# ugadiarov-la-phystech-edu/OCRL

Hardware: AMD Instinct MI355X
Metric: images/sec (node) SLATE pretrain 128x128, 6 slots, 3 iters (higher is better)
Workload: dtype f32

## Files before the change

include/ocrl_hip.h:

```cpp
#ifndef OCRL_HIP_H
#define OCRL_HIP_H
#include <stddef.h>

#ifdef __cplusplus
extern "C" {
#endif

#define OCRL_ABI_VERSION 5

const char* ocrl_last_error(void);
int ocrl_abi_version(void);

typedef struct ocrl_slate ocrl_slate;
typedef struct ocrl_slate_config {
    int obs_size, obs_channels;
    int vocab_size, d_model;
    int cnn_hidden;
    int num_slots, num_iterations, slot_size, mlp_hidden;
    int num_dec_blocks, num_dec_heads;
    float dropout;
    int max_batch;
    int use_bcdec;
    int hard;
    int num_slot_heads;
// ... 1 lines not shown

size_t ocrl_slate_config_size(void);
int ocrl_slate_create(const ocrl_slate_config* cfg, ocrl_slate** out);
void ocrl_slate_destroy(ocrl_slate* h);

int ocrl_slate_param_count(const ocrl_slate* h);
int ocrl_slate_param_info(const ocrl_slate* h, int i, char* name, int name_cap, int shape[4], int* ndim,
                          long long* offset, long long* numel, int* group);
long long ocrl_slate_flat_size(const ocrl_slate* h);
long long ocrl_slate_group_begin(const ocrl_slate* h, int group);
size_t ocrl_slate_workspace_bytes(const ocrl_slate* h);

int ocrl_slate_bind(ocrl_slate* h, float* params, float* grads, float* adam_m, float* adam_v, void* workspace, size_t workspace_bytes);

int ocrl_slate_forward(ocrl_slate* h, const float* obs, int B, float tau, int train, unsigned long long seed,
                       const float* noise_z, const float* noise_zh, const float* noise_slots, void* stream);
int ocrl_slate_backward(ocrl_slate* h, void* stream);
int ocrl_slate_encode(ocrl_slate* h, const float* obs, int B, unsigned long long seed, const float* noise_slots, void* stream);
int ocrl_slate_encode_backward(ocrl_slate* h, const float* dslots, void* stream);
int ocrl_slate_freeze_weights(ocrl_slate* h, int on);
int ocrl_slate_generate(ocrl_slate* h, void* stream);
int ocrl_slate_clip_adam(ocrl_slate* h, const float lr[3], float clip, int step, float grad_scale, void* stream);
int ocrl_slate_grad_norm(ocrl_slate* h, void* stream);
float* ocrl_slate_metrics(const ocrl_slate* h);
int ocrl_slate_tensor(const ocrl_slate* h, const char* name, float** ptr, long long* count);
int ocrl_slate_soft_z(ocrl_slate* h, void* stream);
int ocrl_slate_dropout_mask(const ocrl_slate* h, unsigned site, long long n, float* out, void* stream);

int ocrl_gemm(const float* A, const float* B, float* C, int M, int N, int K, int lda, int ldb, int ldc, int akc, int bkc,
              float alpha, const float* bias, int relu, const float* mask, int ldmask, const float* resid, int ldr,
              int splitk, float* ws, void* stream);
typedef struct ocrl_gemm_desc {
    const float* A; const float* B; float* C;
    int M, N, K, lda, ldb, ldc;
    int akc, bkc;
    int batch, batch_inner;
    long long sA, sB, sC, sAi, sBi, sCi;
    int splitk; float alpha;
    const float* bias; int relu;
    float drop_p; unsigned long long drop_seed; unsigned drop_site;
    const float* mask; int ldmask; long long sMask; int mask_elu;
    const float* resid; int ldr; long long sR;
    float adrop_p; unsigned adrop_site; int adrop_ld;
    float* bias_out; long long sBias;
    int a_mode, b_mode; const float* x_lse; const int* x_tok; float x_scale;
    int epi_mode; float* stat; float* hstat; int* hidx; const float* e1; const float* e2; unsigned long long e_seed;
    const float* e_lse; const float* e_rowvec; float e_scale;
    int force_tile, force_sb;
} ocrl_gemm_desc;
size_t ocrl_gemm_desc_size(void);
int ocrl_gemm_ex(const ocrl_gemm_desc* d, float* ws, size_t ws_floats, void* stream);
int ocrl_gemm_plan(const ocrl_gemm_desc* d, int out[6]);
int ocrl_conv2d_fwd(const float* x, const float* w, const float* bias, float* y, int B, int H, int W, int cin, int cin_pad, int ks,
                    int relu, float* ws, void* stream);
int ocrl_conv2d_fwd_lowlat(const float* x, const float* w, const float* bias, float* y, int B, int H, int W, int cin, int cin_pad, int ks,
                           int relu, float* ws, void* stream);
size_t ocrl_conv2d_x3_ws_floats(void);
int ocrl_conv2d_fwd_x3(const float* x, const float* w, const float* bias, float* y, int B, int H, int W, int ks, int relu, float* ws, void* stream);
int ocrl_conv2d_bwd_data_x3(const float* dy, const float* w, const float* mask, float* dx, int B, int H, int W, int ks, float* ws, void* stream);
int ocrl_conv2d_bwd_weight_x3(const float* x, const float* dy, float* dw, int B, int H, int W, int ks, float* ws, size_t ws_floats, void* stream);
int ocrl_conv2d_bwd_data(const float* dy, const float* w, const float* mask, float* dx, int B, int H, int W, int ks, float* ws, void* stream);
size_t ocrl_conv2d_wgrad_ws_floats(int B, int H, int W, int ks, int cin_pad);
int ocrl_conv2d_bwd_weight(const float* x, const float* dy, float* dw, float* db, int B, int H, int W, int cin, int cin_pad, int ks,
                           float* ws, size_t ws_floats, void* stream);
typedef struct ocrl_conv_desc {
    const float* x; const float* w; float* y;
    int B, H, W, cin, cin_pad, ks;
    const float* bias; int relu;
    const float* posmap; const float* mask; int mask_elu;
    int transposed, low_latency;
} ocrl_conv_desc;
size_t ocrl_conv_desc_size(void);
int ocrl_conv2d_ex(const ocrl_conv_desc* d, float* ws, size_t ws_floats, void* stream);
typedef struct ocrl_conv_wgrad_desc {
    const float* x; const float* dy; float* dw; float* db;
    int B, H, W, cin, cin_pad, ks;
    int accumulate;
} ocrl_conv_wgrad_desc;
size_t ocrl_conv_wgrad_desc_size(void);
int ocrl_conv2d_bwd_weight_ex(const ocrl_conv_wgrad_desc* d, float* ws, size_t ws_floats, void* stream);
int ocrl_layernorm_fwd(const float* x, const float* gamma, const float* beta, float* y, float* mean, float* rstd, long long R, int F, void* stream);
int ocrl_layernorm_bwd(const float* dy, const float* x, const float* mean, const float* rstd, const float* gamma, float* dx, float* dgb,
                       long long R, int F, float* ws, size_t ws_floats, void* stream);

int ocrl_sa_input_plan(long long R, int out[3]);
int ocrl_sa_input_fwd(const float* e4, const float* gamma, const float* beta, const float* W0, const float* b0, const float* W2, const float* b2,
                      float* mean, float* rstd, float* h1, float* x, long long R, int max_wgs, void* stream);
int ocrl_sa_input_bwd(const float* dx, const float* h1, const float* e4, const float* mean, const float* rstd, const float* gamma, const float* beta,
                      const float* W0, const float* W2, float* de4, float* dW0, float* db0, float* dW2, float* db2, float* dgamma, float* dbeta,
                      long long R, int max_wgs, float* ws, size_t ws_floats, void* stream);

int ocrl_attention_fwd(const float* q, const float* k, const float* v, float* o, float* lse, int B, int T, int d, int h, int ld,
                       float p, unsigned long long seed, unsigned site, void* stream);
int ocrl_attention_bwd(const float* q, const float* k, const float* v, const float* o, const float* lse, const float* dO,
                       float* dq, float* dk, float* dv, float* delta, int B, int T, int d, int h, int ld,
                       float p, unsigned long long seed, unsigned site, void* stream);

int ocrl_obs_u8_to_f32(const unsigned char* obs_hwc, float* obs_chw, int B, int H, int W, int C, void* stream);

int ocrl_prof_enable(unsigned tag_mask);
int ocrl_prof_collect(double* ms, long long* count, int ntags);

size_t ocrl_slot_attention_ws_floats(int B, int K, int D, int H, int I);
int ocrl_slot_attention_fwd(const float* x, const float* slots0, const float* const* w, float* slots, float* attn, int B, int N, int K, int D,
                            int H, int I, float* ws, size_t ws_floats, void* stream);
int ocrl_slot_attention_bwd(const float* x, const float* dslots, float* dx, float* dslots0, float* const* dw, int B, int N, int K, int D, int H,
                            int I, float* ws, size_t ws_floats, void* stream);
size_t ocrl_slot_attention_mh_ws_floats(int B, int N, int K, int D, int H, int I, int heads);
int ocrl_slot_attention_mh_fwd(const float* x, const float* slots0, const float* const* w, float* slots, float* attn, int B, int N, int K, int D,
                               int H, int I, int heads, float* ws, size_t ws_floats, void* stream);
int ocrl_slot_attention_mh_bwd(const float* x, const float* dslots, float* dx, float* dslots0, float* const* dw, int B, int N, int K, int D, int H,
                               int I, int heads, float* ws, size_t ws_floats, void* stream);
int ocrl_slot_attention_plan(int K, int D, int H, int heads, int* out6);

#define OCRL_POOL_MAX_LAYERS 8
size_t ocrl_pool_transformer_ws_floats(int B, int K, int d, int nhead, int ff, int L);
int ocrl_pool_transformer_fwd(const float* slots, const float* const* w, const float* pos, float* out, int B, int K, int Din, int d, int nhead,
                              int ff, int L, float drop_p, unsigned long long seed, float* ws, size_t ws_floats, void* stream);
int ocrl_pool_transformer_bwd(const float* slots, const float* dout, const float* const* w, float* dslots, float* const* dw, int B, int K, int Din,
                              int d, int nhead, int ff, int L, float drop_p, unsigned long long seed, float* ws, size_t ws_floats, void* stream);
int ocrl_pool_transformer_dropout_mask(int layer, int which, long long n, float drop_p, unsigned long long seed, float* out, void* stream);
size_t ocrl_pool_transformer_long_ws_floats(int B, int K, int Din, int d, int nhead, int ff, int L);
int ocrl_pool_transformer_long_fwd(const float* slots, const float* const* w, const float* pos, float* out, int B, int K, int Din, int d, int nhead,
                                   int ff, int L, float drop_p, unsigned long long seed, float* ws, size_t ws_floats, void* stream);
int ocrl_pool_transformer_long_bwd(const float* slots, const float* dout, const float* const* w, float* dslots, float* const* dw, int B, int K,
                                   int Din, int d, int nhead, int ff, int L, float drop_p, unsigned long long seed, float* ws, size_t ws_floats,
                                   void* stream);

#define OCRL_POOL_RN_MAX_LAYERS 16
size_t ocrl_pool_rn_ws_floats(int B, int K, int D, int ng, const int* g_dims, int nf, const int* f_dims);
int ocrl_pool_rn_fwd(const float* slots, const float* const* w, float* out, int B, int K, int D, int ng, const int* g_dims, int nf, const int* f_dims,
                     float* ws, size_t ws_floats, void* stream);
int ocrl_pool_rn_bwd(const float* slots, const float* dout, const float* const* w, float* dslots, float* const* dw, int B, int K, int D, int ng,
                     const int* g_dims, int nf, const int* f_dims, float* ws, size_t ws_floats, void* stream);

#define OCRL_NATURECNN_MAX_GROUPS 16
#define OCRL_NATURECNN_MAX_CONVS 4
size_t ocrl_naturecnn_ws_floats(int B, int H, int W, int cin, int groups, int cnn_feat_size, int use_cnn_feat, int rep_dim);
int ocrl_naturecnn_fwd(const float* obs, const float* const* w, float* out, int B, int H, int W, int cin, int groups, int cnn_feat_size,
                       int use_cnn_feat, int rep_dim, int save, float* ws, size_t ws_floats, void* stream);
int ocrl_naturecnn_bwd(const float* obs, const float* dout, const float* const* w, float* const* dw, int B, int H, int W, int cin, int groups,
                       int cnn_feat_size, int use_cnn_feat, int rep_dim, float* ws, size_t ws_floats, void* stream);

size_t ocrl_pool_cnn_ws_floats(int B, int H, int W, int D, int rep_dim);
int ocrl_pool_cnn_fwd(const float* tokens, const float* const* w, float* out, int B, int H, int W, int D, int rep_dim, int save, float* ws,
                      size_t ws_floats, void* stream);
int ocrl_pool_cnn_bwd(const float* tokens, const float* dout, const float* const* w, float* dtokens, float* const* dw, int B, int H, int W, int D,
                      int rep_dim, float* ws, size_t ws_floats, void* stream);

#define OCRL_VAE_MAX_STAGES 6
size_t ocrl_vae_ws_floats(int B, int obs_size, int obs_channels, int cnn_feat_size, int latent_dim, int use_cnn_feat, int full);
int ocrl_vae_fwd(const float* obs, const float* const* w, const float* eps, float* rep, float* metrics, float* recon, int B, int obs_size,
                 int obs_channels, int cnn_feat_size, int latent_dim, int use_cnn_feat, float kld_weight, int full, float* ws, size_t ws_floats,
                 void* stream);
int ocrl_vae_bwd(const float* obs, const float* eps, const float* const* w, const float* dloss, const float* drep, float* const* dw, int B,
                 int obs_size, int obs_channels, int cnn_feat_size, int latent_dim, int use_cnn_feat, float kld_weight, int full, float* ws,
                 size_t ws_floats, void* stream);

#define OCRL_MAE_MAX_DEPTH 32
size_t ocrl_mae_ws_floats(int B, int obs_size, int patch, int D, int depth, int heads, int Dd, int ddepth, int dheads, int len_keep, int full);
int ocrl_mae_fwd(const float* obs, const float* const* w, const float* noise, float* rep, float* metrics, float* pred, float* mask,
                 int* ids_restore, int B, int obs_size, int patch, int D, int depth, int heads, int Dd, int ddepth, int dheads, int len_keep,
                 int full, float* ws, size_t ws_floats, void* stream);
int ocrl_mae_bwd(const float* obs, const float* const* w, const float* dloss, const float* drep, float* const* dw, int B, int obs_size,
                 int patch, int D, int depth, int heads, int Dd, int ddepth, int dheads, int len_keep, int full, float* ws, size_t ws_floats,
                 void* stream);
// ... 119 lines not shown
```

ocrl_amd/_lib.py:

```python
import ctypes
import os
from ctypes import POINTER, c_char_p, c_float, c_int, c_longlong, c_size_t, c_uint, c_ulonglong, c_void_p

_HERE = os.path.dirname(os.path.abspath(__file__))
LIB_PATH = os.environ.get("OCRL_HIP_LIB") or os.path.join(_HERE, "libocrl_hip.so")
_lib = None


class SlateConfig(ctypes.Structure):
    _fields_ = [(n, c_int) for n in ("obs_size", "obs_channels", "vocab_size", "d_model", "cnn_hidden", "num_slots",
                                      "num_iterations", "slot_size", "mlp_hidden", "num_dec_blocks", "num_dec_heads")] + \
               [("dropout", c_float), ("max_batch", c_int), ("use_bcdec", c_int), ("hard", c_int), ("num_slot_heads", c_int)]


class IodineConfig(ctypes.Structure):
    _fields_ = [(n, c_int) for n in ("obs_size", "obs_channels", "slot_size", "num_iterations", "num_slots")] + \
               [("sigma", c_float), ("beta", c_float), ("layer_norm", c_int), ("ref_mlp_hidden", c_int), ("max_batch", c_int)]


class GemmDesc(ctypes.Structure):
    _fields_ = [("A", c_void_p), ("B", c_void_p), ("C", c_void_p)] + \
               [(n, c_int) for n in ("M", "N", "K", "lda", "ldb", "ldc", "akc", "bkc", "batch", "batch_inner")] + \
               [(n, c_longlong) for n in ("sA", "sB", "sC", "sAi", "sBi", "sCi")] + \
               [("splitk", c_int), ("alpha", c_float), ("bias", c_void_p), ("relu", c_int),
# ... 51 lines not shown


def conv_desc(**kw):
    d = ConvDesc()
    for k, v in kw.items():
        setattr(d, k, v)
    return d


def conv_wgrad_desc(**kw):
    d = ConvWgradDesc()
    for k, v in kw.items():
        setattr(d, k, v)
    return d


def lib():
    global _lib
    if _lib is not None:
        return _lib
    if not os.path.exists(LIB_PATH):
        raise RuntimeError(
            f"{LIB_PATH} is missing: build it with `python -c 'import __graft_entry__ as g; g.build()'` "
            "(make -C ocrl_amd/csrc).  ocrl_amd has no CPU fallback.")
    import torch
    L = ctypes.CDLL(LIB_PATH)
    p = c_void_p
    L.ocrl_last_error.restype = c_char_p
    L.ocrl_abi_version.restype = c_int
    L.ocrl_slate_config_size.restype = c_size_t
    if L.ocrl_slate_config_size() != ctypes.sizeof(SlateConfig):
        raise RuntimeError(f"libocrl_hip.so: ocrl_slate_config is {L.ocrl_slate_config_size()} bytes, this binding's SlateConfig {ctypes.sizeof(SlateConfig)}")
    L.ocrl_slate_create.argtypes = [POINTER(SlateConfig), POINTER(p)]
    L.ocrl_slate_destroy.argtypes = [p]
    L.ocrl_slate_destroy.restype = None
    L.ocrl_slate_param_count.argtypes = [p]
    L.ocrl_slate_param_info.argtypes = [p, c_int, c_char_p, c_int, POINTER(c_int * 4), POINTER(c_int), POINTER(c_longlong),
                                        POINTER(c_longlong), POINTER(c_int)]
    L.ocrl_slate_flat_size.argtypes = [p]
    L.ocrl_slate_flat_size.restype = c_longlong
    L.ocrl_slate_group_begin.argtypes = [p, c_int]
    L.ocrl_slate_group_begin.restype = c_longlong
    L.ocrl_slate_workspace_bytes.argtypes = [p]
    L.ocrl_slate_workspace_bytes.restype = c_size_t
    L.ocrl_slate_bind.argtypes = [p, p, p, p, p, p, c_size_t]
    L.ocrl_slate_forward.argtypes = [p, p, c_int, c_float, c_int, c_ulonglong, p, p, p, p]
    L.ocrl_slate_backward.argtypes = [p, p]
    L.ocrl_slate_generate.argtypes = [p, p]
    L.ocrl_slate_encode.argtypes = [p, p, c_int, c_ulonglong, p, p]
    L.ocrl_slate_encode_backward.argtypes = [p, p, p]
    L.ocrl_slate_freeze_weights.argtypes = [p, c_int]
    L.ocrl_slate_clip_adam.argtypes = [p, POINTER(c_float * 3), c_float, c_int, c_float, p]
    L.ocrl_slate_grad_norm.argtypes = [p, p]
    L.ocrl_slate_metrics.argtypes = [p]
    L.ocrl_slate_metrics.restype = p
    L.ocrl_slate_tensor.argtypes = [p, c_char_p, POINTER(p), POINTER(c_longlong)]
    L.ocrl_slate_dropout_mask.argtypes = [p, c_uint, c_longlong, p, p]
    L.ocrl_slate_soft_z.argtypes = [p, p]
    L.ocrl_gemm.argtypes = [p, p, p, c_int, c_int, c_int, c_int, c_int, c_int, c_int, c_int, c_float, p, c_int, p, c_int, p, c_int,
                            c_int, p, p]
    L.ocrl_gemm_desc_size.restype = c_size_t
    L.ocrl_gemm_ex.argtypes = [POINTER(GemmDesc), p, c_size_t, p]
    L.ocrl_gemm_plan.argtypes = [POINTER(GemmDesc), POINTER(c_int * 6)]
    L.ocrl_conv2d_fwd.argtypes = [p, p, p, p, c_int, c_int, c_int, c_int, c_int, c_int, c_int, p, p]
    L.ocrl_conv2d_fwd_lowlat.argtypes = [p, p, p, p, c_int, c_int, c_int, c_int, c_int, c_int, c_int, p, p]
    L.ocrl_conv2d_x3_ws_floats.restype = c_size_t
    L.ocrl_conv2d_fwd_x3.argtypes = [p, p, p, p, c_int, c_int, c_int, c_int, c_int, p, p]
    L.ocrl_conv2d_bwd_data_x3.argtypes = [p, p, p, p, c_int, c_int, c_int, c_int, p, p]
    L.ocrl_conv2d_bwd_weight_x3.argtypes = [p, p, p, c_int, c_int, c_int, c_int, p, c_size_t, p]
    L.ocrl_conv2d_bwd_data.argtypes = [p, p, p, p, c_int, c_int, c_int, c_int, p, p]
    L.ocrl_conv2d_wgrad_ws_floats.argtypes = [c_int, c_int, c_int, c_int, c_int]
    L.ocrl_conv2d_wgrad_ws_floats.restype = c_size_t
    L.ocrl_conv2d_bwd_weight.argtypes = [p, p, p, p, c_int, c_int, c_int, c_int, c_int, c_int, p, c_size_t, p]
    L.ocrl_conv_desc_size.restype = c_size_t
    L.ocrl_conv_wgrad_desc_size.restype = c_size_t
    for name, cls in (("ocrl_conv_desc", ConvDesc), ("ocrl_conv_wgrad_desc", ConvWgradDesc)):
        n = getattr(L, name + "_size")()
        if n != ctypes.sizeof(cls):
            raise RuntimeError(f"libocrl_hip.so: {name} is {n} bytes, this binding's {cls.__name__} {ctypes.sizeof(cls)}")
    L.ocrl_conv2d_ex.argtypes = [POINTER(ConvDesc), p, c_size_t, p]
    L.ocrl_conv2d_bwd_weight_ex.argtypes = [POINTER(ConvWgradDesc), p, c_size_t, p]
    L.ocrl_layernorm_fwd.argtypes = [p, p, p, p, p, p, c_longlong, c_int, p]
    L.ocrl_layernorm_bwd.argtypes = [p, p, p, p, p, p, p, c_longlong, c_int, p, c_size_t, p]
    L.ocrl_sa_input_plan.argtypes = [c_longlong, POINTER(c_int * 3)]
    L.ocrl_sa_input_fwd.argtypes = [p] * 11 + [c_longlong, c_int, p]
    L.ocrl_sa_input_bwd.argtypes = [p] * 16 + [c_longlong, c_int, p, c_size_t, p]
    L.ocrl_attention_fwd.argtypes = [p, p, p, p, p, c_int, c_int, c_int, c_int, c_int, c_float, c_ulonglong, c_uint, p]
    L.ocrl_attention_bwd.argtypes = [p, p, p, p, p, p, p, p, p, p, c_int, c_int, c_int, c_int, c_int, c_float, c_ulonglong, c_uint, p]
    L.ocrl_obs_u8_to_f32.argtypes = [p, p, c_int, c_int, c_int, c_int, p]
    L.ocrl_prof_enable.argtypes = [c_uint]
    L.ocrl_prof_collect.argtypes = [POINTER(ctypes.c_double * 8), POINTER(c_longlong * 8), c_int]
    L.ocrl_iodine_create.argtypes = [POINTER(IodineConfig), POINTER(p)]
    L.ocrl_iodine_destroy.argtypes = [p]
    L.ocrl_iodine_destroy.restype = None
    L.ocrl_iodine_param_count.argtypes = [p]
    L.ocrl_iodine_param_info.argtypes = [p, c_int, c_char_p, c_int, POINTER(c_int * 4), POINTER(c_int), POINTER(c_longlong), POINTER(c_longlong)]
    L.ocrl_iodine_flat_size.argtypes = [p]
    L.ocrl_iodine_flat_size.restype = c_longlong
    L.ocrl_iodine_workspace_bytes.argtypes = [p]
    L.ocrl_iodine_workspace_bytes.restype = c_size_t
    L.ocrl_iodine_bind.argtypes = [p, p, p, p, p, p, c_size_t]
    L.ocrl_iodine_forward.argtypes = [p, p, c_int, c_ulonglong, p, p]
    L.ocrl_iodine_backward.argtypes = [p, p]
    L.ocrl_iodine_clip_adam.argtypes = [p, c_float, c_float, c_int, c_float, p]
    L.ocrl_iodine_grad_norm.argtypes = [p, p]
    L.ocrl_iodine_metrics.argtypes = [p]
    L.ocrl_iodine_metrics.restype = p
    L.ocrl_iodine_tensor.argtypes = [p, c_char_p, POINTER(p), POINTER(c_longlong)]
    L.ocrl_slot_attention_ws_floats.argtypes = [c_int, c_int, c_int, c_int, c_int]
    L.ocrl_slot_attention_ws_floats.restype = c_size_t
    L.ocrl_slot_attention_fwd.argtypes = [p, p, POINTER(p), p, p, c_int, c_int, c_int, c_int, c_int, c_int, p, c_size_t, p]
    L.ocrl_slot_attention_bwd.argtypes = [p, p, p, p, POINTER(p), c_int, c_int, c_int, c_int, c_int, c_int, p, c_size_t, p]
    L.ocrl_slot_attention_mh_ws_floats.argtypes = [c_int] * 7
    L.ocrl_slot_attention_mh_ws_floats.restype = c_size_t
    L.ocrl_slot_attention_mh_fwd.argtypes = [p, p, POINTER(p), p, p] + [c_int] * 7 + [p, c_size_t, p]
    L.ocrl_slot_attention_mh_bwd.argtypes = [p, p, p, p, POINTER(p)] + [c_int] * 7 + [p, c_size_t, p]
    L.ocrl_slot_attention_plan.argtypes = [c_int, c_int, c_int, c_int, POINTER(c_int * 6)]
    L.ocrl_pool_transformer_ws_floats.argtypes = [c_int, c_int, c_int, c_int, c_int, c_int]
    L.ocrl_pool_transformer_ws_floats.restype = c_size_t
    L.ocrl_pool_transformer_fwd.argtypes = [p, POINTER(p), p, p, c_int, c_int, c_int, c_int, c_int, c_int, c_int, c_float, c_ulonglong, p, c_size_t, p]
    L.ocrl_pool_transformer_bwd.argtypes = [p, p, POINTER(p), p, POINTER(p), c_int, c_int, c_int, c_int, c_int, c_int, c_int, c_float, c_ulonglong, p,
                                            c_size_t, p]
    L.ocrl_pool_transformer_dropout_mask.argtypes = [c_int, c_int, c_longlong, c_float, c_ulonglong, p, p]
    L.ocrl_pool_transformer_long_ws_floats.argtypes = [c_int] * 7
    L.ocrl_pool_transformer_long_ws_floats.restype = c_size_t
    L.ocrl_pool_transformer_long_fwd.argtypes = L.ocrl_pool_transformer_fwd.argtypes
    L.ocrl_pool_transformer_long_bwd.argtypes = L.ocrl_pool_transformer_bwd.argtypes
    L.ocrl_pool_rn_ws_floats.argtypes = [c_int, c_int, c_int, c_int, POINTER(c_int), c_int, POINTER(c_int)]
    L.ocrl_pool_rn_ws_floats.restype = c_size_t
    L.ocrl_pool_rn_fwd.argtypes = [p, POINTER(p), p, c_int, c_int, c_int, c_int, POINTER(c_int), c_int, POINTER(c_int), p, c_size_t, p]
    L.ocrl_pool_rn_bwd.argtypes = [p, p, POINTER(p), p, POINTER(p), c_int, c_int, c_int, c_int, POINTER(c_int), c_int, POINTER(c_int), p, c_size_t, p]
    L.ocrl_naturecnn_ws_floats.argtypes = [c_int] * 8
    L.ocrl_naturecnn_ws_floats.restype = c_size_t
    L.ocrl_naturecnn_fwd.argtypes = [p, POINTER(p), p] + [c_int] * 9 + [p, c_size_t, p]
    L.ocrl_naturecnn_bwd.argtypes = [p, p, POINTER(p), POINTER(p)] + [c_int] * 8 + [p, c_size_t, p]
    L.ocrl_pool_cnn_ws_floats.argtypes = [c_int] * 5
    L.ocrl_pool_cnn_ws_floats.restype = c_size_t
    L.ocrl_pool_cnn_fwd.argtypes = [p, POINTER(p), p] + [c_int] * 6 + [p, c_size_t, p]
    L.ocrl_pool_cnn_bwd.argtypes = [p, p, POINTER(p), p, POINTER(p)] + [c_int] * 5 + [p, c_size_t, p]
    L.ocrl_vae_ws_floats.argtypes = [c_int] * 7
    L.ocrl_vae_ws_floats.restype = c_size_t
    L.ocrl_vae_fwd.argtypes = [p, POINTER(p), p, p, p, p] + [c_int] * 6 + [c_float, c_int, p, c_size_t, p]
    L.ocrl_vae_bwd.argtypes = [p, p, POINTER(p), p, p, POINTER(p)] + [c_int] * 6 + [c_float, c_int, p, c_size_t, p]
    L.ocrl_mae_ws_floats.argtypes = [c_int] * 11
    L.ocrl_mae_ws_floats.restype = c_size_t
    L.ocrl_mae_fwd.argtypes = [p, POINTER(p), p, p, p, p, p, p] + [c_int] * 11 + [p, c_size_t, p]
    L.ocrl_mae_bwd.argtypes = [p, POINTER(p), p, p, POINTER(p)] + [c_int] * 11 + [p, c_size_t, p]
    L.ocrl_mae_rank.argtypes = [p, p, p, p, c_int, c_int, c_int, p]
    L.ocrl_probe_ws_floats.argtypes = [c_int] * 7 + [POINTER(c_int), c_int]
    L.ocrl_probe_ws_floats.restype = c_size_t
    L.ocrl_probe_fwd.argtypes = [p, POINTER(p), p, p, p, p, p] + [c_int] * 8 + [POINTER(c_int), c_float, c_int, POINTER(c_int), POINTER(c_int),
                                 POINTER(c_int), p, c_size_t, p]
    L.ocrl_probe_bwd.argtypes = [p, p, POINTER(p), POINTER(p)] + [c_int] * 7 + [POINTER(c_int), c_float, c_int, p, c_size_t, p]
    L.ocrl_probe_match_ws_floats.argtypes = [c_int, c_int]
    L.ocrl_probe_match_ws_floats.restype = c_size_t
    L.ocrl_probe_match.argtypes = [p, c_int, c_longlong, p, p, p, p, p, p] + [c_int] * 6 + [POINTER(c_int)] * 3 + [p, c_size_t, p]
    L.ocrl_ari_counts.argtypes = [p, c_longlong, c_longlong, c_longlong, c_int, p, c_longlong, c_longlong, c_longlong, c_int, c_int, c_int, c_longlong, p, p, p]
    L.ocrl_acnet_desc_size.restype = c_size_t
    if L.ocrl_acnet_desc_size() != ctypes.sizeof(AcnetDesc):
        raise RuntimeError(f"libocrl_hip.so: ocrl_acnet_desc is {L.ocrl_acnet_desc_size()} bytes, this binding's AcnetDesc {ctypes.sizeof(AcnetDesc)}")
    L.ocrl_acnet_ws_floats.argtypes = [POINTER(AcnetDesc)]
    L.ocrl_acnet_ws_floats.restype = c_size_t
    L.ocrl_acnet_fwd.argtypes = [POINTER(AcnetDesc), p, POINTER(p), p, p, p, p, c_int, p, c_size_t, p]
    L.ocrl_acnet_bwd.argtypes = [POINTER(AcnetDesc), p, POINTER(p), p, p, p, p, p, POINTER(p), p, c_size_t, p]
    L.ocrl_acnet_ppo_fwd_bwd.argtypes = [POINTER(AcnetDesc), p, POINTER(p), p, p, p, p, c_float, c_float, c_float, c_int, p, p, POINTER(p), p, c_size_t, p]
    L.ocrl_acnet_a2c_fwd_bwd.argtypes = [POINTER(AcnetDesc), p, POINTER(p), p, p, p, c_float, c_float, c_int, p, p, POINTER(p), p, c_size_t, p]
# ... 48 lines not shown
```

ocrl_amd/csrc/capi.cpp:

```cpp
#include <stdarg.h>
#include <stdint.h>
#include <string.h>

#include <new>

#include "../../include/ocrl_hip.h"
#include "iodine_model.h"
#include "slate_model.h"

static thread_local char g_err[512] = "";

void ocrl_set_error(const char* fmt, ...) {
    va_list ap;
    va_start(ap, fmt);
    vsnprintf(g_err, sizeof g_err, fmt, ap);
    va_end(ap);
}

template <class M>
struct Handle {
    using Model = M;
    M* m = nullptr;
};
struct ocrl_slate : Handle<SlateModel> {};
// ... 193 lines not shown
    if (conv_pack_x3_launch(w, ws, nullptr, ST(stream), ks)) return 1;
    ConvArgs a;
    a.X = x; a.Y = y; a.B = B; a.H = H; a.W = W; a.bias = bias; a.relu = relu;
    return conv_x3_launch(a, ws, ST(stream), ks);
}
int ocrl_conv2d_bwd_data_x3(const float* dy, const float* w, const float* mask, float* dx, int B, int H, int W, int ks, float* ws, void* stream) {
    if (ks != 3 && ks != 5) { ocrl_set_error("ocrl_conv2d_bwd_data_x3: ks must be 3 or 5"); return 1; }
    if (conv_pack_x3_launch(w, ws, ws + conv_x3_pack_floats(5), ST(stream), ks)) return 1;
    ConvArgs a;
    a.X = dy; a.Y = dx; a.B = B; a.H = H; a.W = W; a.mask = mask;
    return conv_x3_launch(a, ws + conv_x3_pack_floats(5), ST(stream), ks);
}
int ocrl_conv2d_bwd_data(const float* dy, const float* w, const float* mask, float* dx, int B, int H, int W, int ks, float* ws, void* stream) {
    float* bw = ws + (size_t)ks * ks * 64 * 64;
    if (conv_pack_launch(w, ws, bw, ks, 64, 64, 64, ST(stream))) return 1;
    ConvArgs a;
    a.X = dy; a.Wp = bw; a.Y = dx; a.B = B; a.H = H; a.W = W; a.mask = mask;
    return conv_fwd_launch(a, ks, 64, 64, ST(stream));
}
size_t ocrl_conv2d_wgrad_ws_floats(int B, int H, int W, int ks, int cin_pad) { return conv_wgrad_ws_floats(B, H, W, ks, cin_pad) + (1 << 16); }
int ocrl_conv2d_bwd_weight(const float* x, const float* dy, float* dw, float* db, int B, int H, int W, int cin, int cin_pad, int ks, float* ws,
                           size_t ws_floats, void* stream) {
    if (ws_floats < ocrl_conv2d_wgrad_ws_floats(B, H, W, ks, cin_pad)) { ocrl_set_error("ocrl_conv2d_bwd_weight: workspace too small"); return 1; }
    WgradArgs a;
    a.X = x; a.dY = dy; a.part = ws; a.B = B; a.H = H; a.W = W;
    if (conv_wgrad_launch(a, ks, cin_pad, 64, cin, dw, 0, ST(stream), 0)) return 1;
    if (db) return colsum_launch(dy, 64, db, (long long)B * H * W, 64, 0, 1.f, ws, ws_floats, ST(stream));
    return 0;
}
int ocrl_conv2d_bwd_weight_x3(const float* x, const float* dy, float* dw, int B, int H, int W, int ks, float* ws, size_t ws_floats, void* stream) {
    if (ks != 3 && ks != 5) { ocrl_set_error("ocrl_conv2d_bwd_weight_x3: ks must be 3 or 5"); return 1; }
    if (ws_floats < ocrl_conv2d_wgrad_ws_floats(B, H, W, ks, 64)) { ocrl_set_error("ocrl_conv2d_bwd_weight_x3: workspace too small"); return 1; }
    WgradArgs a;
    a.X = x; a.dY = dy; a.part = ws; a.B = B; a.H = H; a.W = W;
    return conv_wgrad_launch(a, ks, 64, 64, 64, dw, 0, ST(stream), 1);
}
static bool conv_kernel_built(int ks, int cin_pad) { return (ks == 5 && (cin_pad == 64 || cin_pad == 8)) || (ks == 3 && cin_pad == 64); }
static bool aligned16(const void* p) { return ((uintptr_t)p & 15) == 0; }
size_t ocrl_conv_desc_size(void) { return sizeof(ocrl_conv_desc); }
int ocrl_conv2d_ex(const ocrl_conv_desc* d, float* ws, size_t ws_floats, void* stream) {
    if (!d) { ocrl_set_error("ocrl_conv2d_ex: null descriptor"); return 1; }
    if (!d->x || !d->w || !d->y || !ws || d->B < 1 || d->H < 1 || d->W < 1) { ocrl_set_error("ocrl_conv2d_ex: x, w, y, ws and a non-empty image are required"); return 1; }
    if (!conv_kernel_built(d->ks, d->cin_pad)) { ocrl_set_error("ocrl_conv2d_ex: no kernel for ks=%d cin_pad=%d (built: 5/64, 5/8, 3/64)", d->ks, d->cin_pad); return 1; }
    if (d->cin < 1 || d->cin > d->cin_pad) { ocrl_set_error("ocrl_conv2d_ex: cin %d outside 1 .. cin_pad %d", d->cin, d->cin_pad); return 1; }
    if (d->relu < 0 || d->relu > 2) { ocrl_set_error("ocrl_conv2d_ex: relu must be 0, 1 (ReLU) or 2 (ELU), got %d", d->relu); return 1; }
    if (d->mask_elu && !d->mask) { ocrl_set_error("ocrl_conv2d_ex: mask_elu needs a mask"); return 1; }
    if (d->transposed && (d->cin != 64 || d->cin_pad != 64)) { ocrl_set_error("ocrl_conv2d_ex: the transposed (backward-data) form needs cin = cin_pad = 64"); return 1; }
    if (!aligned16(d->x) || !aligned16(d->y) || !aligned16(ws) || !aligned16(d->bias) || !aligned16(d->posmap) || !aligned16(d->mask)) {
        ocrl_set_error("ocrl_conv2d_ex: x, y, ws, bias, posmap and mask must be 16-byte aligned");
        return 1;
    }
    const size_t pack = (size_t)d->ks * d->ks * d->cin_pad * 64, need = d->transposed ? 2 * pack : pack;
    if (ws_floats < need) { ocrl_set_error("ocrl_conv2d_ex: workspace of %zu floats, %zu needed", ws_floats, need); return 1; }
    float* bw = d->transposed ? ws + pack : nullptr;
    if (conv_pack_launch(d->w, ws, bw, d->ks, d->cin_pad, 64, d->cin, ST(stream))) return 1;
    ConvArgs a;
    a.X = d->x; a.Wp = bw ? bw : ws; a.Y = d->y; a.B = d->B; a.H = d->H; a.W = d->W; a.bias = d->bias; a.relu = d->relu;
    a.posmap = d->posmap; a.mask = d->mask; a.mask_elu = d->mask_elu ? 1 : 0;
    return conv_fwd_launch(a, d->ks, d->cin_pad, 64, ST(stream), d->low_latency ? 1 : 0);
}
size_t ocrl_conv_wgrad_desc_size(void) { return sizeof(ocrl_conv_wgrad_desc); }
int ocrl_conv2d_bwd_weight_ex(const ocrl_conv_wgrad_desc* d, float* ws, size_t ws_floats, void* stream) {
    if (!d) { ocrl_set_error("ocrl_conv2d_bwd_weight_ex: null descriptor"); return 1; }
    if (!d->x || !d->dy || !d->dw || !ws || d->B < 1 || d->H < 1 || d->W < 1) { ocrl_set_error("ocrl_conv2d_bwd_weight_ex: x, dy, dw, ws and a non-empty image are required"); return 1; }
    if (!conv_kernel_built(d->ks, d->cin_pad)) { ocrl_set_error("ocrl_conv2d_bwd_weight_ex: no kernel for ks=%d cin_pad=%d (built: 5/64, 5/8, 3/64)", d->ks, d->cin_pad); return 1; }
    if (d->cin < 1 || d->cin > d->cin_pad) { ocrl_set_error("ocrl_conv2d_bwd_weight_ex: cin %d outside 1 .. cin_pad %d", d->cin, d->cin_pad); return 1; }
    if (!aligned16(d->x) || !aligned16(d->dy) || !aligned16(ws)) { ocrl_set_error("ocrl_conv2d_bwd_weight_ex: x, dy and ws must be 16-byte aligned"); return 1; }
    const size_t need = ocrl_conv2d_wgrad_ws_floats(d->B, d->H, d->W, d->ks, d->cin_pad);
    if (ws_floats < need) { ocrl_set_error("ocrl_conv2d_bwd_weight_ex: workspace of %zu floats, %zu needed", ws_floats, need); return 1; }
    const int acc = d->accumulate ? 1 : 0;
    WgradArgs a;
    a.X = d->x; a.dY = d->dy; a.part = ws; a.B = d->B; a.H = d->H; a.W = d->W;
    if (conv_wgrad_launch(a, d->ks, d->cin_pad, 64, d->cin, d->dw, acc, ST(stream), 0)) return 1;
    if (d->db) return colsum_launch(d->dy, 64, d->db, (long long)d->B * d->H * d->W, 64, acc, 1.f, ws, ws_floats, ST(stream));
    return 0;
}
int ocrl_layernorm_fwd(const float* x, const float* g, const float* b, float* y, float* mean, float* rstd, long long R, int F, void* stream) {
    return layernorm_fwd_launch(x, g, b, y, mean, rstd, R, F, ST(stream));
}
int ocrl_layernorm_bwd(const float* dy, const float* x, const float* mean, const float* rstd, const float* g, float* dx, float* dgb, long long R,
                       int F, float* ws, size_t ws_floats, void* stream) {
    return layernorm_bwd_launch(dy, x, mean, rstd, g, dx, dgb, R, F, 0, 0, ws, ws_floats, ST(stream));
}

int ocrl_sa_input_plan(long long R, int out[3]) {
    if (!out || R <= 0) { ocrl_set_error("ocrl_sa_input_plan: needs R > 0 and an output array"); return 1; }
    sa_input_plan(R, 0, out);
    return 0;
}
int ocrl_sa_input_fwd(const float* e4, const float* gamma, const float* beta, const float* W0, const float* b0, const float* W2, const float* b2,
                      float* mean, float* rstd, float* h1, float* x, long long R, int max_wgs, void* stream) {
    return sa_input_fwd_launch(e4, gamma, beta, W0, b0, W2, b2, mean, rstd, nullptr, h1, x, R, max_wgs, ST(stream));
}
int ocrl_sa_input_bwd(const float* dx, const float* h1, const float* e4, const float* mean, const float* rstd, const float* gamma, const float* beta,
                      const float* W0, const float* W2, float* de4, float* dW0, float* db0, float* dW2, float* db2, float* dgamma, float* dbeta,
                      long long R, int max_wgs, float* ws, size_t ws_floats, void* stream) {
    return sa_input_bwd_launch(dx, h1, e4, mean, rstd, gamma, beta, W0, W2, de4, dW0, db0, dW2, db2, dgamma, dbeta, R, max_wgs, ws, ws_floats,
                               ST(stream));
}

int ocrl_attention_fwd(const float* q, const float* k, const float* v, float* o, float* lse, int B, int T, int d, int h, int ld, float p,
                       unsigned long long seed, unsigned site, void* stream) {
    AttnArgs a;
    a.q = q; a.k = k; a.v = v; a.o = o; a.lse = lse; a.B = B; a.T = T; a.d = d; a.h = h; a.ld = ld; a.p = p; a.seed = seed; a.site = site;
    return attn_launch(a, 0, ST(stream));
}
int ocrl_attention_bwd(const float* q, const float* k, const float* v, const float* o, const float* lse, const float* dO, float* dq,
                       float* dk, float* dv, float* delta, int B, int T, int d, int h, int ld, float p, unsigned long long seed,
                       unsigned site, void* stream) {
    AttnArgs a;
    a.q = q; a.k = k; a.v = v; a.o = const_cast<float*>(o); a.lse = const_cast<float*>(lse); a.B = B; a.T = T; a.d = d; a.h = h; a.ld = ld;
    a.p = p; a.seed = seed; a.site = site; a.dO = dO; a.dq = dq; a.dk = dk; a.dv = dv; a.delta = delta;
    return attn_launch(a, 1, ST(stream));
}


int ocrl_iodine_create(const ocrl_iodine_config* c, ocrl_iodine** out) {
    if (!c || !out) { ocrl_set_error("ocrl_iodine_create: null argument"); return 1; }
    if (c->obs_size < 16 || c->obs_size % 16 || c->obs_channels != 3 || c->slot_size < 4 || c->slot_size % 4 || c->slot_size > 256 ||
        c->num_iterations < 1 || c->num_slots < 1 || c->num_slots > 16 || c->ref_mlp_hidden < 64 || c->ref_mlp_hidden % 64 || c->max_batch < 1 ||
        !(c->sigma > 0.f)) {
        ocrl_set_error("ocrl_iodine_create: invalid configuration");
        return 1;
    }
    IodineConfig k;
    k.obs_size = c->obs_size; k.obs_channels = c->obs_channels; k.slot_size = c->slot_size; k.num_iters = c->num_iterations;
    k.num_slots = c->num_slots; k.sigma = c->sigma; k.beta = c->beta; k.layer_norm = c->layer_norm; k.ref_mlp_hidden = c->ref_mlp_hidden;
    k.max_batch = c->max_batch;
    return h_create(k, out);
}
void ocrl_iodine_destroy(ocrl_iodine* h) { h_destroy(h); }
int ocrl_iodine_param_count(const ocrl_iodine* h) { return h_param_count(h); }
int ocrl_iodine_param_info(const ocrl_iodine* h, int i, char* name, int name_cap, int shape[4], int* ndim, long long* offset, long long* numel) {
    return h_param_info(h, i, name, name_cap, shape, ndim, offset, numel, nullptr);
}
long long ocrl_iodine_flat_size(const ocrl_iodine* h) { return h_flat_size(h); }
size_t ocrl_iodine_workspace_bytes(const ocrl_iodine* h) { return h_workspace_bytes(h); }
int ocrl_iodine_bind(ocrl_iodine* h, float* p, float* g, float* m, float* v, void* ws, size_t n) { return h_bind(h, p, g, m, v, ws, n); }
int ocrl_iodine_forward(ocrl_iodine* h, const float* obs, int B, unsigned long long seed, const float* noise, void* stream) {
    GUARD(h);
    return h->m->forward(obs, B, seed, noise, ST(stream));
}
int ocrl_iodine_backward(ocrl_iodine* h, void* stream) { GUARD(h); return h->m->backward(ST(stream)); }
int ocrl_iodine_clip_adam(ocrl_iodine* h, float lr, float clip, int step, float gscale, void* stream) {
    GUARD(h);
    return h->m->clip_adam(lr, clip, step, gscale, ST(stream));
}
int ocrl_iodine_grad_norm(ocrl_iodine* h, void* stream) { GUARD(h); return h->m->grad_norm(ST(stream)); }
float* ocrl_iodine_metrics(const ocrl_iodine* h) { return h_metrics(h); }
int ocrl_iodine_tensor(const ocrl_iodine* h, const char* name, float** ptr, long long* count) { return h_tensor(h, name, ptr, count); }
}
```

ocrl_amd/csrc/elementwise.hip:

```cpp
#include "common.h"
#include "kernels.h"
#include "layernorm16.h"

#define TINYF 1.17549435e-38f

__device__ inline float block_sum(float v, float* red) {
    v = wave_sum(v);
    const int w = threadIdx.x >> 6, nw = blockDim.x >> 6;
    __syncthreads();
    if ((threadIdx.x & 63) == 0) red[w] = v;
    __syncthreads();
    float s = 0.f;
    for (int i = 0; i < nw; ++i) s += red[i];
    return s;
}
__device__ inline float block_max(float v, float* red) {
    v = wave_max(v);
    const int w = threadIdx.x >> 6, nw = blockDim.x >> 6;
    __syncthreads();
    if ((threadIdx.x & 63) == 0) red[w] = v;
    __syncthreads();
    float s = red[0];
    for (int i = 1; i < nw; ++i) s = fmaxf(s, red[i]);
    return s;
// ... 74 lines not shown
        const int c = i * 64 + lane;
        y[row * F + c] = (v[i] - mu) * rs * g[c] + bta[c];
    }
    if (lane == 0) {
        if (mean) mean[row] = mu;
        if (rstd) rstd[row] = rs;
    }
}

template <int NPL>
__global__ void layernorm_bwd_kernel(const float* __restrict__ dy, const float* __restrict__ x, const float* __restrict__ mean,
                                     const float* __restrict__ rstd, const float* __restrict__ g, float* __restrict__ dx,
                                     float* __restrict__ part, long long R, int accumulate) {
    constexpr int F = 64 * NPL;
    __shared__ float red[4][2 * F];
    const int lane = threadIdx.x & 63, wv = threadIdx.x >> 6;
    float dg[NPL], db[NPL], gg[NPL];
#pragma unroll
    for (int i = 0; i < NPL; ++i) { dg[i] = 0.f; db[i] = 0.f; gg[i] = g[i * 64 + lane]; }
    for (long long row = (long long)blockIdx.x * 4 + wv; row < R; row += (long long)gridDim.x * 4) {
        const float mu = mean[row], rs = rstd[row];
        float xh[NPL], d[NPL];
        float s1 = 0.f, s2 = 0.f;
#pragma unroll
        for (int i = 0; i < NPL; ++i) {
            const int c = i * 64 + lane;
            xh[i] = (x[row * F + c] - mu) * rs;
            const float dyv = dy[row * F + c];
            dg[i] += dyv * xh[i];
            db[i] += dyv;
            d[i] = dyv * gg[i];
            s1 += d[i];
            s2 += d[i] * xh[i];
        }
        s1 = wave_sum(s1) * (1.0f / F);
        s2 = wave_sum(s2) * (1.0f / F);
#pragma unroll
        for (int i = 0; i < NPL; ++i) {
            const int c = i * 64 + lane;
            const float v = rs * (d[i] - s1 - xh[i] * s2);
            dx[row * F + c] = accumulate ? dx[row * F + c] + v : v;
        }
    }
#pragma unroll
    for (int i = 0; i < NPL; ++i) { red[wv][i * 64 + lane] = dg[i]; red[wv][F + i * 64 + lane] = db[i]; }
    __syncthreads();
    for (int c = threadIdx.x; c < 2 * F; c += blockDim.x)
        part[(size_t)blockIdx.x * 2 * F + c] = red[0][c] + red[1][c] + red[2][c] + red[3][c];
}

template <int NV, int NP>
__global__ __launch_bounds__(256) void layernorm16_fwd_kernel(const float* __restrict__ x, const float* __restrict__ g, const float* __restrict__ bta,
                                                              float* __restrict__ y, float* __restrict__ mean, float* __restrict__ rstd, long long R) {
    constexpr int F = 64 * NV;
    const int lane = threadIdx.x & 63, wv = threadIdx.x >> 6, c4 = lane & 15, rsub = lane >> 4;
    const long long row0 = ((long long)blockIdx.x * 4 + wv) * (4 * NP) + rsub;
    float4 v[NP][NV];
#pragma unroll
    for (int i = 0; i < NP; ++i)
#pragma unroll
        for (int k = 0; k < NV; ++k) {
            const long long row = row0 + 4 * i;
            v[i][k] = row < R ? *reinterpret_cast<const float4*>(x + row * F + (k * 16 + c4) * 4) : make_float4(0.f, 0.f, 0.f, 0.f);
        }
    float4 gg[NV], bb[NV];
#pragma unroll
    for (int k = 0; k < NV; ++k) { gg[k] = *reinterpret_cast<const float4*>(g + (k * 16 + c4) * 4); bb[k] = *reinterpret_cast<const float4*>(bta + (k * 16 + c4) * 4); }
#pragma unroll
    for (int i = 0; i < NP; ++i) {
        const long long row = row0 + 4 * i;
        float mu, rs;
        layernorm16_row_fwd<NV>(v[i], mu, rs);
        if (row < R) {
#pragma unroll
            for (int k = 0; k < NV; ++k) *reinterpret_cast<float4*>(y + row * F + (k * 16 + c4) * 4) = layernorm16_affine(v[i][k], rs, gg[k], bb[k]);
            if (c4 == 0) {
                if (mean) mean[row] = mu;
                if (rstd) rstd[row] = rs;
            }
        }
    }
}
template <int NV, int NP>
__global__ __launch_bounds__(256) void layernorm16_bwd_kernel(const float* __restrict__ dy, const float* __restrict__ x, const float* __restrict__ mean,
                                                              const float* __restrict__ rstd, const float* __restrict__ g, float* __restrict__ dx,
                                                              float* __restrict__ part, long long R, int accumulate) {
    constexpr int F = 64 * NV;
    __shared__ float4 red[2][16][16 * NV];
    const int lane = threadIdx.x & 63, wv = threadIdx.x >> 6, c4 = lane & 15, rsub = lane >> 4;
    float4 gg[NV], dg[NV], db[NV];
#pragma unroll
    for (int k = 0; k < NV; ++k) { gg[k] = *reinterpret_cast<const float4*>(g + (k * 16 + c4) * 4); dg[k] = make_float4(0.f, 0.f, 0.f, 0.f); db[k] = dg[k]; }
    for (long long grp = blockIdx.x; grp * (16 * NP) < R; grp += gridDim.x) {
        const long long row0 = (grp * 4 + wv) * (4 * NP) + rsub;
        float4 xv[NP][NV], yv[NP][NV];
        float mu[NP], rs[NP];
#pragma unroll
        for (int i = 0; i < NP; ++i) {
            const long long row = row0 + 4 * i;
            const bool ok = row < R;
#pragma unroll
            for (int k = 0; k < NV; ++k) {
                xv[i][k] = ok ? *reinterpret_cast<const float4*>(x + row * F + (k * 16 + c4) * 4) : make_float4(0.f, 0.f, 0.f, 0.f);
                yv[i][k] = ok ? *reinterpret_cast<const float4*>(dy + row * F + (k * 16 + c4) * 4) : make_float4(0.f, 0.f, 0.f, 0.f);
            }
            mu[i] = ok ? mean[row] : 0.f;
            rs[i] = ok ? rstd[row] : 0.f;
        }
#pragma unroll
        for (int i = 0; i < NP; ++i) {
            const long long row = row0 + 4 * i;
            const Ln16Bwd<NV> r = layernorm16_row_bwd<NV>(xv[i], yv[i], mu[i], rs[i], gg, dg, db);
            if (row < R) {
#pragma unroll
                for (int k = 0; k < NV; ++k) {
                    float4 o = layernorm16_row_dx(r, rs[i], k);
                    float* dp = dx + row * F + (k * 16 + c4) * 4;
                    if (accumulate) { const float4 a = *reinterpret_cast<const float4*>(dp); o.x += a.x; o.y += a.y; o.z += a.z; o.w += a.w; }
                    *reinterpret_cast<float4*>(dp) = o;
                }
            }
        }
    }
#pragma unroll
    for (int k = 0; k < NV; ++k) { red[0][wv * 4 + rsub][k * 16 + c4] = dg[k]; red[1][wv * 4 + rsub][k * 16 + c4] = db[k]; }
    __syncthreads();
    if (threadIdx.x < 32 * NV) {
        const int which = threadIdx.x / (16 * NV), c = threadIdx.x % (16 * NV);
        float4 a = red[which][0][c];
#pragma unroll
        for (int k = 1; k < 16; ++k) { const float4 t = red[which][k][c]; a.x += t.x; a.y += t.y; a.z += t.z; a.w += t.w; }
        *reinterpret_cast<float4*>(part + (size_t)blockIdx.x * (2 * F) + which * F + c * 4) = a;
    }
}

__global__ void colsum_kernel(const float* __restrict__ X, long long ld, float* __restrict__ part, long long R, int F, long long rows_per_chunk) {
    __shared__ float red[4][64];
    const int col = blockIdx.x * 64 + (threadIdx.x & 63), rl = threadIdx.x >> 6;
    const long long r0 = (long long)blockIdx.y * rows_per_chunk;
    const long long r1 = min(R, r0 + rows_per_chunk);
    float s = 0.f;
    if (col < F)
        for (long long r = r0 + rl; r < r1; r += 4) s += X[r * ld + col];
    red[rl][threadIdx.x & 63] = s;
    __syncthreads();
    if (rl == 0 && col < F) part[(size_t)blockIdx.y * F + col] = red[0][threadIdx.x] + red[1][threadIdx.x] + red[2][threadIdx.x] + red[3][threadIdx.x];
}
__global__ __launch_bounds__(256) void colsum4_kernel(const float* __restrict__ X, long long ld, float* __restrict__ part, long long R, int F,
                                                      long long rows_per_chunk) {
    __shared__ float4 red[256];
    const int F4 = F >> 2, RL = 256 / F4;
    const int c4 = threadIdx.x % F4, rl = threadIdx.x / F4;
    const long long r0 = (long long)blockIdx.x * rows_per_chunk;
    const long long r1 = min(R, r0 + rows_per_chunk);
    float4 s0 = make_float4(0.f, 0.f, 0.f, 0.f), s1 = s0, s2 = s0, s3 = s0;
    if (rl < RL) {
        const float* base = X + (size_t)c4 * 4;
        long long r = r0 + rl;
        for (; r + 3 * RL < r1; r += 4 * RL) {
            const float4 a = *reinterpret_cast<const float4*>(base + r * ld), b = *reinterpret_cast<const float4*>(base + (r + RL) * ld);
            const float4 c = *reinterpret_cast<const float4*>(base + (r + 2 * RL) * ld), d = *reinterpret_cast<const float4*>(base + (r + 3 * RL) * ld);
            s0.x += a.x; s0.y += a.y; s0.z += a.z; s0.w += a.w;
            s1.x += b.x; s1.y += b.y; s1.z += b.z; s1.w += b.w;
            s2.x += c.x; s2.y += c.y; s2.z += c.z; s2.w += c.w;
            s3.x += d.x; s3.y += d.y; s3.z += d.z; s3.w += d.w;
        }
        for (; r < r1; r += RL) {
            const float4 a = *reinterpret_cast<const float4*>(base + r * ld);
            s0.x += a.x; s0.y += a.y; s0.z += a.z; s0.w += a.w;
        }
    }
    red[threadIdx.x] = make_float4(s0.x + s1.x + s2.x + s3.x, s0.y + s1.y + s2.y + s3.y, s0.z + s1.z + s2.z + s3.z, s0.w + s1.w + s2.w + s3.w);
    __syncthreads();
    if (threadIdx.x < F4) {
        float4 t = red[threadIdx.x];
        for (int k = 1; k < RL; ++k) { const float4 v = red[k * F4 + threadIdx.x]; t.x += v.x; t.y += v.y; t.z += v.z; t.w += v.w; }
        *reinterpret_cast<float4*>(part + (size_t)blockIdx.x * F + threadIdx.x * 4) = t;
    }
}
__global__ __launch_bounds__(256) void colsum_final_kernel(const float* __restrict__ part, float* __restrict__ out, int nchunk, int F, int accumulate, float scale) {
    __shared__ float red[16][16];
    const int cl = threadIdx.x & 15, rl = threadIdx.x >> 4;
    const int c = blockIdx.x * 16 + cl;
    float s0 = 0.f, s1 = 0.f;
    if (c < F) {
        int k = rl;
        for (; k + 16 < nchunk; k += 32) { s0 += part[(size_t)k * F + c]; s1 += part[(size_t)(k + 16) * F + c]; }
        if (k < nchunk) s0 += part[(size_t)k * F + c];
    }
    red[rl][cl] = s0 + s1;
    __syncthreads();
    if (rl == 0 && c < F) {
        float t = 0.f;
#pragma unroll
        for (int k = 0; k < 16; ++k) t += red[k][cl];
        t *= scale;
        out[c] = accumulate ? out[c] + t : t;
    }
}

__global__ void reduce_partials_kernel(const float* __restrict__ part, int n, float* __restrict__ out, float scale, int accumulate) {
    __shared__ float red[4];
    float s = 0.f;
    for (int i = threadIdx.x; i < n; i += blockDim.x) s += part[i];
    s = block_sum(s, red);
    if (threadIdx.x == 0) out[0] = (accumulate ? out[0] : 0.f) + s * scale;
}

__global__ void mse_kernel(const float* __restrict__ obs, const float* __restrict__ recon, float* __restrict__ drecon,
                           float* __restrict__ part, int B, int C, int H, int W, float inv_b) {
    __shared__ float red[4];
    const long long n = (long long)B * H * W, hw = (long long)H * W;
    float s = 0.f;
    for (long long i = (long long)blockIdx.x * blockDim.x + threadIdx.x; i < n; i += (long long)gridDim.x * blockDim.x) {
        const long long b = i / hw, r = i % hw;
        const float4 rc = *reinterpret_cast<const float4*>(recon + i * 4);
        const float rv[4] = {rc.x, rc.y, rc.z, rc.w};
        float d[4] = {0.f, 0.f, 0.f, 0.f};
        for (int c = 0; c < C; ++c) {
            const float e = rv[c] - obs[(b * C + c) * hw + r];
            s += e * e;
            d[c] = 2.f * e * inv_b;
        }
        if (drecon) *reinterpret_cast<float4*>(drecon + i * 4) = make_float4(d[0], d[1], d[2], d[3]);
    }
    s = block_sum(s, red);
    if (threadIdx.x == 0) part[blockIdx.x] = s;
}

#define GS_MAXPT 16
template <int NPT>
__global__ __launch_bounds__(256) void gumbel_softmax_kernel(const float* __restrict__ raw, const float* __restrict__ e1,
                                                             const float* __restrict__ e2, float* __restrict__ z,
                                                             int* __restrict__ tokens, int V, float inv_tau,
                                                             unsigned long long seed, float* __restrict__ zst) {
    __shared__ float red[4];
    __shared__ float redv[4];
    __shared__ int redi[4];
    const long long row = blockIdx.x;
    const float* r = raw + row * V;
    const int npt = NPT ? NPT : V / 256;
    float x[GS_MAXPT];
    float mx = -INFINITY;
#pragma unroll
    for (int i = 0; i < GS_MAXPT; ++i)
        if (i < npt) { x[i] = r[i * 256 + threadIdx.x]; mx = fmaxf(mx, x[i]); }
    mx = block_max(mx, red);
    float s = 0.f;
#pragma unroll
    for (int i = 0; i < GS_MAXPT; ++i)
        if (i < npt) s += __expf(x[i] - mx);
    s = block_sum(s, red);
    const float lse = mx + __logf(s);
    float u[GS_MAXPT];
    float best = -INFINITY;
    int besti = 0;
    float m2 = -INFINITY;
#pragma unroll
    for (int i = 0; i < GS_MAXPT; ++i)
        if (i < npt) {
            const int v = i * 256 + threadIdx.x;
            const float lp = x[i] - lse;
            float ea, eb;
            if (e1) { ea = e1[row * V + v]; eb = e2[row * V + v]; }
            else {
                const uint64_t idx = (uint64_t)row * V + v;
                const uint2 ba = rng_bits4(seed, SITE_GUMBEL_Z, idx);
                ea = -__logf(u01_24(ba.x));
                eb = -__logf(u01_24(ba.y));
            }
            const float g1 = -__logf(ea + TINYF), g2 = -__logf(eb + TINYF);
            u[i] = (lp + g1) * inv_tau;
            m2 = fmaxf(m2, u[i]);
            const float h = (lp + g2) * inv_tau;
            if (h > best) { best = h; besti = v; }
        }
    m2 = block_max(m2, red);
    float s2 = 0.f;
#pragma unroll
    for (int i = 0; i < GS_MAXPT; ++i)
        if (i < npt) { u[i] = __expf(u[i] - m2); s2 += u[i]; }
// ... 741 lines not shown
    if (tid < dh) qs[tid] = base[(size_t)t * ld + tid] * scale;
    __syncthreads();
    float mx = -INFINITY;
    for (int j = tid; j < nk; j += 256) {
        const float* kr = base + (size_t)j * ld + d;
        float a = 0.f;
        for (int c = 0; c < dh; c += 4) {
            const float4 kv = *reinterpret_cast<const float4*>(kr + c);
            a += qs[c] * kv.x + qs[c + 1] * kv.y + qs[c + 2] * kv.z + qs[c + 3] * kv.w;
        }
        sc[j] = a;
        mx = fmaxf(mx, a);
    }
    red[tid] = mx;
    __syncthreads();
    block_tree_max<256>(red);
    mx = red[0];
    __syncthreads();
    float sum = 0.f;
    for (int j = tid; j < nk; j += 256) { const float e = __expf(sc[j] - mx); sc[j] = e; sum += e; }
    red[tid] = sum;
    __syncthreads();
    block_tree_sum<256>(red);
    const float inv = 1.0f / red[0];
    __syncthreads();
    const int nsl = 256 / dh, c = tid % dh, sl = tid / dh;
    float acc = 0.f;
    if (sl < nsl)
        for (int j = sl; j < nk; j += nsl) acc += sc[j] * base[(size_t)j * ld + 2 * d + c];
    red[tid] = sl < nsl ? acc : 0.f;
    __syncthreads();
    if (tid < dh) {
        float a = 0.f;
        for (int k = 0; k < nsl; ++k) a += red[k * dh + tid];
        out[(size_t)b * d + hd * dh + tid] = a * inv;
    }
}

__global__ void onehot_kernel(const int* __restrict__ tokens, float* __restrict__ z, long long n, int V) {
    const long long i = (long long)blockIdx.x * blockDim.x + threadIdx.x;
    if (i >= n) return;
    z[i] = (int)(i % V) == tokens[i / V] ? 1.f : 0.f;
}

int nchw_to_nhwc8_launch(const float* in, float* out, int B, int C, int H, int W, hipStream_t st) {
    OCRL_REQUIRE(C <= 8, "nchw_to_nhwc8: C must be <= 8");
    const long long n = (long long)B * H * W;
    hipLaunchKernelGGL(nchw_to_nhwc8_kernel, GRID1D(n), 0, st, in, out, B, C, H, W);
    OCRL_CHECK_LAUNCH("nchw_to_nhwc8");
    return 0;
}
int patchify4_launch(const float* in, float* out, int B, int C, int S, hipStream_t st) {
    OCRL_REQUIRE(S % 4 == 0, "patchify4: S %% 4 != 0");
    const long long n = (long long)B * (S / 4) * (S / 4) * C * 4;
    hipLaunchKernelGGL(patchify4_kernel, GRID1D(n), 0, st, in, out, B, C, S);
    OCRL_CHECK_LAUNCH("patchify4");
    return 0;
}
int pixel_shuffle_launch(const float* in, float* out, int B, int h, int w, int Cout, int forward, const float* mask, hipStream_t st) {
    const long long n = (long long)B * h * w * Cout;
    hipLaunchKernelGGL(pixel_shuffle_kernel, GRID1D(n), 0, st, in, out, B, h, w, Cout, forward, mask);
    OCRL_CHECK_LAUNCH("pixel_shuffle");
    return 0;
}
int layernorm_fwd_launch(const float* x, const float* g, const float* b, float* y, float* mean, float* rstd, long long R, int F, hipStream_t st) {
    OCRL_REQUIRE(F % 64 == 0 && F >= 64 && F <= 256, "layernorm: F must be 64..256, multiple of 64 (got %d)", F);
    dim3 grid(cdiv(R, 4)), blk(256);
    const bool al16 = aligned16(x, y, g, b);
    switch (F / 64) {
        case 1:
            if (al16) hipLaunchKernelGGL((layernorm16_fwd_kernel<1, 4>), dim3((unsigned)cdiv(R, 64)), blk, 0, st, x, g, b, y, mean, rstd, R);
            else hipLaunchKernelGGL(layernorm_fwd_kernel<1>, grid, blk, 0, st, x, g, b, y, mean, rstd, R);
            break;
        case 2: hipLaunchKernelGGL(layernorm_fwd_kernel<2>, grid, blk, 0, st, x, g, b, y, mean, rstd, R); break;
        case 3:
            if (al16) hipLaunchKernelGGL((layernorm16_fwd_kernel<3, 2>), dim3((unsigned)cdiv(R, 32)), blk, 0, st, x, g, b, y, mean, rstd, R);
            else hipLaunchKernelGGL(layernorm_fwd_kernel<3>, grid, blk, 0, st, x, g, b, y, mean, rstd, R);
            break;
        default: hipLaunchKernelGGL(layernorm_fwd_kernel<4>, grid, blk, 0, st, x, g, b, y, mean, rstd, R); break;
    }
    OCRL_CHECK_LAUNCH("layernorm_fwd");
    return 0;
}
int colsum_launch(const float* X, long long ld, float* out, long long R, int F, int accumulate, float scale, float* ws, size_t ws_floats, hipStream_t st) {
    if (F % 4 == 0 && ld % 4 == 0 && F <= 1024 && F >= 4 && (((uintptr_t)X) & 15) == 0 && R >= 1024) {
        long long nchunk = 2048;
        if (nchunk > R / 8) nchunk = R / 8;
        if ((size_t)nchunk * F > ws_floats) nchunk = (long long)(ws_floats / F);
        if (nchunk >= 16) {
            const long long rpc = (R + nchunk - 1) / nchunk;
            nchunk = (R + rpc - 1) / rpc;
            hipLaunchKernelGGL(colsum4_kernel, dim3((unsigned)nchunk), dim3(256), 0, st, X, ld, ws, R, F, rpc);
            OCRL_CHECK_LAUNCH("colsum4");
            hipLaunchKernelGGL(colsum_final_kernel, dim3(cdiv(F, 16)), dim3(256), 0, st, ws, out, (int)nchunk, F, accumulate, scale);
            OCRL_CHECK_LAUNCH("colsum_final");
            return 0;
        }
    }
    const int cb = cdiv(F, 64);
    long long nchunk = 1024 / cb;
    if (nchunk < 1) nchunk = 1;
    if (nchunk > (R + 63) / 64) nchunk = (R + 63) / 64;
    if (nchunk < 1) nchunk = 1;
    OCRL_REQUIRE((size_t)nchunk * F <= ws_floats, "colsum: workspace too small (%lld x %d)", nchunk, F);
    const long long rpc = (R + nchunk - 1) / nchunk;
    hipLaunchKernelGGL(colsum_kernel, dim3(cb, (int)nchunk), dim3(256), 0, st, X, ld, ws, R, F, rpc);
    OCRL_CHECK_LAUNCH("colsum");
    hipLaunchKernelGGL(colsum_final_kernel, dim3(cdiv(F, 16)), dim3(256), 0, st, ws, out, (int)nchunk, F, accumulate, scale);
    OCRL_CHECK_LAUNCH("colsum_final");
    return 0;
}
int layernorm_bwd_launch(const float* dy, const float* x, const float* mean, const float* rstd, const float* g, float* dx,
                         float* dgb, long long R, int F, int accumulate_dx, int accumulate_dgb, float* ws, size_t ws_floats, hipStream_t st) {
    OCRL_REQUIRE(F % 64 == 0 && F >= 64 && F <= 256, "layernorm bwd: F must be 64..256, multiple of 64 (got %d)", F);
    int nblk = (int)((R + 3) / 4);
    if (nblk > 2048) nblk = 2048;
    while (nblk > 64 && (size_t)nblk * 2 * F * 2 + (size_t)8 * 2 * F > ws_floats) nblk /= 2;
    const size_t need = (size_t)nblk * 2 * F;
    OCRL_REQUIRE(need + (size_t)8 * 2 * F <= ws_floats, "layernorm bwd: workspace too small");
    dim3 grid(nblk), blk(256);
    const bool al16 = aligned16(x, dy, dx, g, ws);
    switch (F / 64) {
        case 1:
            if (al16) hipLaunchKernelGGL((layernorm16_bwd_kernel<1, 4>), grid, blk, 0, st, dy, x, mean, rstd, g, dx, ws, R, accumulate_dx);
            else hipLaunchKernelGGL(layernorm_bwd_kernel<1>, grid, blk, 0, st, dy, x, mean, rstd, g, dx, ws, R, accumulate_dx);
            break;
        case 2: hipLaunchKernelGGL(layernorm_bwd_kernel<2>, grid, blk, 0, st, dy, x, mean, rstd, g, dx, ws, R, accumulate_dx); break;
        case 3:
            if (al16) hipLaunchKernelGGL((layernorm16_bwd_kernel<3, 2>), grid, blk, 0, st, dy, x, mean, rstd, g, dx, ws, R, accumulate_dx);
            else hipLaunchKernelGGL(layernorm_bwd_kernel<3>, grid, blk, 0, st, dy, x, mean, rstd, g, dx, ws, R, accumulate_dx);
            break;
        default: hipLaunchKernelGGL(layernorm_bwd_kernel<4>, grid, blk, 0, st, dy, x, mean, rstd, g, dx, ws, R, accumulate_dx); break;
    }
    OCRL_CHECK_LAUNCH("layernorm_bwd");
    return colsum_launch(ws, 2 * F, dgb, nblk, 2 * F, accumulate_dgb, 1.f, ws + need, ws_floats - need, st);
}
int reduce_partials_launch(const float* part, int n, float* out, float scale, int accumulate, hipStream_t st) {
    hipLaunchKernelGGL(reduce_partials_kernel, dim3(1), dim3(256), 0, st, part, n, out, scale, accumulate);
    OCRL_CHECK_LAUNCH("reduce_partials");
    return 0;
}
int mse_launch(const float* obs, const float* recon, float* drecon, float* out, int B, int C, int H, int W, float* ws, size_t ws_floats, hipStream_t st) {
    OCRL_REQUIRE(C <= 4, "mse: C must be <= 4");
    const int nblk = 1024;
    OCRL_REQUIRE(ws_floats >= (size_t)nblk, "mse: workspace too small");
    hipLaunchKernelGGL(mse_kernel, dim3(nblk), dim3(256), 0, st, obs, recon, drecon, ws, B, C, H, W, 1.0f / B);
    OCRL_CHECK_LAUNCH("mse");
    return reduce_partials_launch(ws, nblk, out, 1.0f / B, 0, st);
}
int gumbel_softmax_launch(const float* raw, const float* e1, const float* e2, float* z, int* tokens, long long R, int V, float tau,
                          unsigned long long seed, hipStream_t st, float* zst) {
    OCRL_REQUIRE(V % 256 == 0 && V <= 256 * GS_MAXPT, "gumbel_softmax: V must be a multiple of 256, <= %d", 256 * GS_MAXPT);
    OCRL_REQUIRE((e1 == nullptr) == (e2 == nullptr), "gumbel_softmax: give both noise tensors or none");
    switch (V / 256) {
        case 16: hipLaunchKernelGGL(gumbel_softmax_kernel<16>, dim3((unsigned)R), dim3(256), 0, st, raw, e1, e2, z, tokens, V, 1.0f / tau, seed, zst); break;
        case 8: hipLaunchKernelGGL(gumbel_softmax_kernel<8>, dim3((unsigned)R), dim3(256), 0, st, raw, e1, e2, z, tokens, V, 1.0f / tau, seed, zst); break;
        default: hipLaunchKernelGGL(gumbel_softmax_kernel<0>, dim3((unsigned)R), dim3(256), 0, st, raw, e1, e2, z, tokens, V, 1.0f / tau, seed, zst); break;
    }
    OCRL_CHECK_LAUNCH("gumbel_softmax");
    return 0;
}
int softmax_bwd_rows_launch(const float* z, float* d, long long R, int V, float scale, hipStream_t st) {
    OCRL_REQUIRE(V % 256 == 0 && V <= 256 * GS_MAXPT, "softmax_bwd_rows: V must be a multiple of 256, <= %d", 256 * GS_MAXPT);
    if (V == 4096) hipLaunchKernelGGL(softmax_bwd_rows_kernel<16>, dim3((unsigned)R), dim3(256), 0, st, z, d, V, scale);
    else hipLaunchKernelGGL(softmax_bwd_rows_kernel<0>, dim3((unsigned)R), dim3(256), 0, st, z, d, V, scale);
    OCRL_CHECK_LAUNCH("softmax_bwd_rows");
    return 0;
}
int softmax_stat_combine_launch(const float* stat, int nseg, long long R, float* lse, const float* hstat, const int* hidx, int* tokens,
                                const float* pred, int ldp, const int* tok, float* out, float scale, float* ws, size_t ws_floats, hipStream_t st,
                                const float* cdf_scores, int cdf_V, float cdf_tau, unsigned long long cdf_seed) {
    OCRL_REQUIRE(nseg >= 1 && nseg <= 64, "softmax_stat_combine: 1..64 segments (got %d)", nseg);
    const long long nblk = (R + 15) / 16;
    OCRL_REQUIRE(!pred || (tok && out && ws && ws_floats >= (size_t)nblk), "softmax_stat_combine: cross-entropy needs tokens, an output and %lld workspace floats", nblk);
    CdfArgs cdf;
    cdf.scores = cdf_scores; cdf.V = cdf_V; cdf.tau = cdf_tau; cdf.seed = cdf_seed;
    OCRL_REQUIRE(!cdf_scores || (hstat && hidx && tokens && cdf_V > 0 && cdf_V <= nseg * 64), "softmax_stat_combine: inverse-CDF sampling arguments");
    hipLaunchKernelGGL(softmax_stat_combine_kernel, dim3((unsigned)nblk), dim3(1024), 0, st, stat, nseg, R, lse, hstat, hidx, tokens, pred, ldp, tok,
                       pred ? ws : nullptr, cdf);
    OCRL_CHECK_LAUNCH("softmax_stat_combine");
    if (pred) return reduce_partials_launch(ws, (int)nblk, out, scale, 0, st);
    return 0;
}
int exp_rows_launch(const float* y, const float* lse, float* z, long long R, int V, hipStream_t st) {
    OCRL_REQUIRE(V % 4 == 0, "exp_rows: V %% 4 != 0");
    const long long n4 = R * (V / 4);
    hipLaunchKernelGGL(exp_rows_kernel, dim3((unsigned)((n4 + 255) / 256)), dim3(256), 0, st, y, lse, z, n4, V / 4);
    OCRL_CHECK_LAUNCH("exp_rows");
    return 0;
}
int rowdot_bias64_launch(const float* g, const float* act, const float* bias, long long R, float* out, hipStream_t st) {
    OCRL_REQUIRE(((((uintptr_t)g) | ((uintptr_t)act) | ((uintptr_t)bias)) & 15) == 0, "rowdot: operands must be 16-byte aligned");
    hipLaunchKernelGGL(rowdot_bias64_kernel, dim3((unsigned)((R + 15) / 16)), dim3(256), 0, st, g, act, bias, R, out);
    OCRL_CHECK_LAUNCH("rowdot_bias64");
    return 0;
}
int embed_fwd_launch(const int* tokens, const float* dict, const float* bos, const float* pe, float* out, int B, int T, int d, float p,
                     unsigned long long seed, hipStream_t st) {
    OCRL_REQUIRE(d % 4 == 0, "embed: d %% 4 != 0");
    const long long n = (long long)B * T * (d / 4);
    hipLaunchKernelGGL(embed_fwd_kernel, dim3((unsigned)cdiv(n, 1024)), dim3(256), 0, st, tokens, dict, bos, pe, out, B, T, d, p, seed);
    OCRL_CHECK_LAUNCH("embed_fwd");
    return 0;
}
static size_t eb_align(size_t n) { return (n + 63) & ~(size_t)63; }
size_t embed_bwd_ws_floats(long long BT, int V, int d) {
    const size_t nchunk = (size_t)cdiv(BT, EB_CHUNK), nunit = (size_t)cdiv(BT, EB_UNIT);
    return eb_align(nchunk * (V + 1)) + 2 * eb_align((size_t)V + 2) + eb_align((size_t)BT) + eb_align(nunit * 2 * d);
}
int embed_bwd_launch(float* g, const int* tokens, float* ddict, int B, int T, int V, int d, float p, unsigned long long seed, float* ws,
                     size_t ws_floats, hipStream_t st) {
    const long long BT = (long long)B * T;
    OCRL_REQUIRE(d % 4 == 0 && d <= 1024 && V + 1 <= 16384 && BT < (1ll << 31), "embed_bwd: unsupported shape (d %d, vocabulary %d, %lld rows)", d, V, BT);
    OCRL_REQUIRE(ws && ws_floats >= embed_bwd_ws_floats(BT, V, d), "embed_bwd: scratch too small");
    const int nchunk = cdiv(BT, EB_CHUNK), nunit = cdiv(BT, EB_UNIT);
    int* hist = reinterpret_cast<int*>(ws);
    int* total = hist + eb_align((size_t)nchunk * (V + 1));
    int* base = total + eb_align((size_t)V + 2);
// ... 179 lines not shown
```

ocrl_amd/csrc/kernels.h:

```cpp
#pragma once
#include "common.h"
#include "../../include/ocrl_hip.h"

enum { PROF_CONV5 = 0, PROF_CONV_OTHER = 1, PROF_WGRAD = 2, PROF_GEMM = 3, PROF_SA_FWD = 4, PROF_SA_BWD = 5, PROF_ATTN_FWD = 6, PROF_ATTN_BWD = 7, PROF_NTAGS = 8 };
int prof_begin(int tag, hipStream_t st);
void prof_end(int idx, hipStream_t st);

struct GemmArgs {
    const float* A = nullptr;
    const float* B = nullptr;
    float* C = nullptr;
    int M = 0, N = 0, K = 0;
    int lda = 0, ldb = 0, ldc = 0;
    int akc = 1, bkc = 1;
    int batch = 1;
    int batch_inner = 1;
    long long sA = 0, sB = 0, sC = 0;
    long long sAi = 0, sBi = 0, sCi = 0;
    int splitk = 1;
    long long sCsplit = 0;
    float alpha = 1.f;
    const float* bias = nullptr;
    int relu = 0;
    float drop_p = 0.f;
// ... 121 lines not shown
struct PcDxArgs {
    const float* dY = nullptr; const float* Wd = nullptr; float* dX = nullptr;
    int H = 0, W = 0, D = 0, OH = 0, OW = 0, HB = 0, WT = 0, Dp = 0, passes = 0, upw = 0;
    long long units = 0, groups = 0;
};
int pc_conv1_fwd_launch(const float* X, const float* w, const float* bias, float* Wp, float* Y, int B, int H, int W, int D, hipStream_t st);
int pc_conv1_dw_launch(const float* X, const float* dY, float* part, int B, int H, int W, int D, hipStream_t st);
int pc_conv1_dw_reduce_launch(const float* part, float* dw, float* db, int B, int H, int W, int D, hipStream_t st);
int pc_conv1_dx_launch(const float* dY, const float* w, float* Wd, float* dX, int B, int H, int W, int D, hipStream_t st);

#define PROBE_MAX_SLOTS 12
#define PROBE_MAX_PROPS 8
#define PROBE_MAX_WIDTH 256
struct ProbeSchema { int P; int t[PROBE_MAX_PROPS], a[PROBE_MAX_PROPS], b[PROBE_MAX_PROPS], kind[PROBE_MAX_PROPS]; };
int probe_schema_check(const ProbeSchema& sc, int T, int O);
int probe_match_check(int B, int K, int N, int T, int O);
int probe_match_launch(const float* out, int ld_row, long long ld_img, const float* y, const float* dloss, float* cost, int* col, float* part,
                       float* metrics, float* dout, int B, int K, int N, int T, int O, const ProbeSchema& sc, hipStream_t st);
int probe_leaky_fwd_launch(float* x, long long n, float slope, hipStream_t st);
int probe_leaky_bwd_launch(float* dx, const float* h, long long n, float slope, hipStream_t st);

int vae_permute_launch(const float* src, float* dst, long long R, int C, int HW, int rows, int pack, hipStream_t st);
int vae_pad_rows_launch(const float* src, float* dst, int rows, int rows_pad, int K, hipStream_t st);
int vae_kl_fwd_launch(const float* ml, const float* eps, float* latent, float* part, float* rep, int B, int L, hipStream_t st);
int vae_loss_launch(const float* part, float* metrics, int B, float kld_weight, hipStream_t st);
int vae_kl_bwd_launch(const float* ml, const float* eps, const float* dlat, const float* drep, const float* dloss, float* dml, int B, int L,
                      float kld_weight, hipStream_t st);
int vae_scale_launch(const float* x, float* y, const float* g, long long n, hipStream_t st);
int vae_recon_nchw_launch(const float* r4, float* out, int B, int C, int HW, hipStream_t st);

#define MAE_MAX_PATCHES 1024
int mae_rank_launch(const float* noise, int* restore, int* keep, float* mask, int* restore_out, float* mask_out, int B, int L, int len_keep,
                    hipStream_t st);
int mae_patch_gather_launch(const float* obs, const int* ids, float* out, int B, int n, int S, int p, hipStream_t st);
int mae_tokens_fwd_launch(const float* embed, const float* cls, const float* pos, const int* ids, float* x0, int B, int n, int D, hipStream_t st);
int mae_tokens_bwd_launch(const float* dx0, float* dembed, float* dcls, int B, int n, int D, hipStream_t st);
int mae_unshuffle_fwd_launch(const float* e, const float* mtok, const float* dpos, const int* restore, float* xd, int B, int L, int len_keep, int Dd,
                             hipStream_t st);
int mae_unshuffle_bwd_launch(const float* dxd, const int* keep, const float* mask, float* de, float* dmtok, float* part, int B, int L, int len_keep,
                             int Dd, hipStream_t st);
int mae_gelu_fwd_launch(const float* pre, float* y, long long n, hipStream_t st);
int mae_gelu_bwd_launch(const float* dy, const float* pre, float* dpre, long long n, hipStream_t st);
int mae_ln_fwd_launch(const float* x, const float* g, const float* b, float* y, float* mean, float* rstd, long long R, int F, float eps, hipStream_t st);
int mae_ln_chunks(long long R);
int mae_ln_bwd_launch(const float* dy, const float* x, const float* mean, const float* rstd, const float* g, const float* resid, float* dx, float* dg,
                      float* db, float* part, long long R, int F, hipStream_t st);
int mae_loss_launch(const float* pred, const float* obs, const float* mask, const float* dloss, float* part, float* loss, float* dpred, int B, int L,
                    int len_keep, int S, int p, hipStream_t st);

struct ConvArgs {
    const float* X = nullptr;
    const float* Wp = nullptr;
    float* Y = nullptr;
    int B = 0, H = 0, W = 0;
    const float* bias = nullptr;
    int relu = 0;
    const float* posmap = nullptr;
    const float* mask = nullptr;
    int mask_elu = 0;
};
size_t conv_x3_pack_floats(int KS = 5);
int conv_pack_x3_launch(const float* W, float* fwd3, float* bwd3, hipStream_t st, int KS = 5);
int conv_x3_launch(const ConvArgs& a, const float* pack3, hipStream_t st, int KS = 5);
struct WgradArgs;
int conv_wgrad_x3_stage(const WgradArgs& a, int nchunk, hipStream_t st, int KS = 5);
struct WgradArgs {
    const float* X = nullptr;
    const float* dY = nullptr;
    float* part = nullptr;
    int B = 0, H = 0, W = 0;
};
int conv_fwd_launch(const ConvArgs& a, int KS, int CIN, int COUT, hipStream_t st, int low_latency = 0);
int conv_wgrad_launch(const WgradArgs& a, int KS, int CIN, int COUT, int cin_real, float* dW, int accumulate, hipStream_t st, int x3 = -1);
size_t conv_wgrad_ws_floats(int B, int H, int W, int KS, int CIN);
int conv_pack_launch(const float* W, float* fwd, float* bwd, int KS, int CIN, int COUT, int cin_real, hipStream_t st);

int nchw_to_nhwc8_launch(const float* in, float* out, int B, int C, int H, int W, hipStream_t st);
int patchify4_launch(const float* in, float* out, int B, int C, int S, hipStream_t st);
int pixel_shuffle_launch(const float* in, float* out, int B, int h, int w, int Cout, int forward, const float* mask, hipStream_t st);
int layernorm_fwd_launch(const float* x, const float* g, const float* b, float* y, float* mean, float* rstd, long long R, int F, hipStream_t st);
int layernorm_bwd_launch(const float* dy, const float* x, const float* mean, const float* rstd, const float* g, float* dx,
                         float* dgb, long long R, int F, int accumulate_dx, int accumulate_dgb, float* ws, size_t ws_floats, hipStream_t st);
int colsum_launch(const float* X, long long ld, float* out, long long R, int F, int accumulate, float scale, float* ws, size_t ws_floats, hipStream_t st);

#define SA_INPUT_SLAB (2 * 4096 + 4 * 64)
void sa_input_plan(long long R, int max_wgs, int out[3]);
int sa_input_fwd_launch(const float* e4, const float* gamma, const float* beta, const float* W0, const float* b0, const float* W2, const float* b2,
                        float* mean, float* rstd, float* ln0, float* h1, float* x, long long R, int max_wgs, hipStream_t st);
int sa_input_bwd_launch(const float* dx, const float* h1, const float* e4, const float* mean, const float* rstd, const float* gamma, const float* beta,
                        const float* W0, const float* W2, float* de4, float* dW0, float* db0, float* dW2, float* db2, float* dgamma, float* dbeta,
                        long long R, int max_wgs, float* ws, size_t ws_floats, hipStream_t st);
int reduce_partials_launch(const float* part, int n, float* out, float scale, int accumulate, hipStream_t st);
int mse_launch(const float* obs, const float* recon, float* drecon, float* out, int B, int C, int H, int W, float* ws, size_t ws_floats, hipStream_t st);
int gumbel_softmax_launch(const float* raw, const float* e1, const float* e2, float* z, int* tokens, long long R, int V, float tau,
                          unsigned long long seed, hipStream_t st, float* zst = nullptr);
int softmax_bwd_rows_launch(const float* z, float* d, long long R, int V, float scale, hipStream_t st);
int softmax_stat_combine_launch(const float* stat, int nseg, long long R, float* lse, const float* hstat, const int* hidx, int* tokens,
                                const float* pred, int ldp, const int* tok, float* out, float scale, float* ws, size_t ws_floats, hipStream_t st,
                                const float* cdf_scores = nullptr, int cdf_V = 0, float cdf_tau = 1.f, unsigned long long cdf_seed = 0);
int exp_rows_launch(const float* y, const float* lse, float* z, long long R, int V, hipStream_t st);
int rowdot_bias64_launch(const float* g, const float* act, const float* bias, long long R, float* out, hipStream_t st);
int embed_fwd_launch(const int* tokens, const float* dict, const float* bos, const float* pe, float* out, int B, int T, int d, float p,
                     unsigned long long seed, hipStream_t st);
size_t embed_bwd_ws_floats(long long BT, int V, int d);
int embed_bwd_launch(float* g, const int* tokens, float* ddict, int B, int T, int V, int d, float p, unsigned long long seed, float* ws,
                     size_t ws_floats, hipStream_t st);
int dropout_apply_launch(const float* x, float* y, long long n, float p, unsigned long long seed, unsigned site, hipStream_t st);
int dropout_mask_launch(float* y, long long n, float p, unsigned long long seed, unsigned site, hipStream_t st);
int cross_attn_fwd_launch(const float* Q, const float* Km, const float* Vm, float* O, float* P, int B, int T, int K, int d, int h, float p,
                          unsigned long long seed, unsigned site, hipStream_t st);
size_t cross_attn_bwd_ws_floats(int B, int T, int K, int d, int h);
int cross_attn_bwd_launch(const float* dO, const float* Q, const float* Km, const float* Vm, const float* P, float* dQ, float* dKm, float* dVm,
                          int B, int T, int K, int d, int h, float p, unsigned long long seed, unsigned site, float* part, size_t part_floats,
                          hipStream_t st);
int obs_u8_to_f32_launch(const unsigned char* in, float* out, int B, int H, int W, int C, hipStream_t st);
int fill_launch(float* x, long long n, float v, hipStream_t st);
int axpy_launch(const float* x, float* y, long long n, float a, hipStream_t st);
int posmap_launch(const float* Wpos, const float* bpos, float* out, int S, int C, hipStream_t st);
int posgrid_launch(float* out, int S, hipStream_t st);
int im2col5_launch(const float* x8, float* col, long long npix, int H, int W, int C, int ldc, hipStream_t st);
int unpack5_launch(const float* dWp, float* dW, int C, int ldc, hipStream_t st);
int pad_cols_launch(const float* in, int ldi, float* out, int ldo, long long R, int C, int Cout, hipStream_t st);

bool xattn_supported(int K, int d, int h);
int xattn_kp(int K, int h);
struct XaFoldHost {
    const float* mem = nullptr;
    const float* Wq[8]; const float* Wk[8]; const float* Wv[8]; const float* Wo[8];
    float* ck[8]; float* cv[8];
    float* Ab[8]; float* AbT[8]; float* Vo[8]; float* VoT[8];
    int B = 0, K = 0, d = 0, h = 0, nblk = 0;
};
int xattn_fold_fwd_launch(const XaFoldHost& f, hipStream_t st);
struct XaHost {
    const float* x = nullptr;
    const float* resid = nullptr;
    float* y = nullptr;
    float* P = nullptr;
    const float *Ab = nullptr, *AbT = nullptr, *Vo = nullptr, *VoT = nullptr;
    const float* gd = nullptr;
    float *Pd = nullptr, *dS = nullptr;
    int B = 0, T = 0, K = 0, d = 0, h = 0;
    float p = 0.f; unsigned long long seed = 0; unsigned site_p = 0, site_o = 0;
};
int xattn_launch(const XaHost& h, int backward, hipStream_t st);


struct SaWts {
    int ln_in_g, ln_in_b, ln_s_g, ln_s_b, ln_m_g, ln_m_b;
    int Wq, WqT, Wk, WkT, Wv, WvT, Wih, WihT, Whh, WhhT, bih, bhh, W0, W0T, b0, W2, W2T, b2;
    int total;
};
static inline SaWts sa_wts_layout(int C, int D, int H) {
    SaWts o; int a = 0;
    auto take = [&](int n) { int r = a; a += (n + 3) & ~3; return r; };
    o.ln_in_g = take(C); o.ln_in_b = take(C); o.ln_s_g = take(D); o.ln_s_b = take(D); o.ln_m_g = take(D); o.ln_m_b = take(D);
    o.Wq = take(D * D); o.WqT = take(D * D); o.Wk = take(D * C); o.WkT = take(C * D); o.Wv = take(D * C); o.WvT = take(C * D);
    o.Wih = take(3 * D * D); o.WihT = take(3 * D * D); o.Whh = take(3 * D * D); o.WhhT = take(3 * D * D);
    o.bih = take(3 * D); o.bhh = take(3 * D);
    o.W0 = take(H * D); o.W0T = take(H * D); o.b0 = take(H); o.W2 = take(D * H); o.W2T = take(D * H); o.b2 = take(D);
    o.total = a;
    return o;
}
struct SaSave { int sprev, sn, q, u, r, z, n, hn, sg, m, hid, qp, up, upn, csum, ld; };
static inline SaSave sa_save_layout(int C, int D, int H, int NH = 1) {
    SaSave o;
// ... 118 lines not shown
```

ocrl_amd/csrc/slate_model.cpp:

```cpp
#include "slate_model.h"

#include <stdlib.h>

#include <math.h>
#include <stdarg.h>
#include <string.h>

static std::string fmt(const char* f, ...) {
    char buf[256];
    va_list ap;
    va_start(ap, f);
    vsnprintf(buf, sizeof buf, f, ap);
    va_end(ap);
    return buf;
}

SlateModel::SlateModel(const SlateConfig& c) : cfg(c) {
    S = c.obs_size; E = S / 4; T = E * E; N = S * S; V = c.vocab; d = c.d_model; C = c.cnn_hidden;
    K = c.num_slots; I = c.num_iters; D = c.slot_size; H = c.mlp_hidden; NB = c.num_blocks; NH = c.num_heads;
    DH = d / NH; Bmax = c.max_batch; SH = c.slot_heads > 0 ? c.slot_heads : 1;
    const int ch = c.obs_channels;
    add_param("_dvae._encoder.0.m.weight", {64, ch, 4, 4}, 0); add_param("_dvae._encoder.0.m.bias", {64}, 0);
    for (int i = 1; i < 7; ++i) { add_param(fmt("_dvae._encoder.%d.m.weight", i), {64, 64, 1, 1}, 0); add_param(fmt("_dvae._encoder.%d.m.bias", i), {64}, 0); }
    add_param("_dvae._encoder.7.weight", {V, 64, 1, 1}, 0); add_param("_dvae._encoder.7.bias", {V}, 0);
// ... 157 lines not shown
    if (cfg.use_bcdec) {
        const size_t BKN = BK * (size_t)N;
        bc_Wc_ = carve(nullptr, 25 * 64 * 5 + 64); bc_W1r_ = carve(nullptr, (size_t)25 * 64 * D); bc_P1_ = carve(nullptr, (size_t)N * 64);
        bc_M_ = carve(nullptr, BK * 1600); bc_T_ = carve(nullptr, BK * 1600);
        bc_c1_ = carve("bc_c1", BKN * 64); bc_c2_ = carve("bc_c2", BKN * 64); bc_c3_ = carve("bc_c3", BKN * 64);
        bc_out4_ = carve(nullptr, BKN * 4); bc_dout4_ = carve(nullptr, BKN * 4);
        bc_gA_ = carve(nullptr, BKN * 64); bc_gB_ = carve(nullptr, BKN * 64);
        for (int i = 0; i < 2; ++i) {
            bc_pk_[i] = carve(nullptr, 25 * 64 * 64); bc_pkb_[i] = carve(nullptr, 25 * 64 * 64);
            if (conv_x3_ > 0) {
                float* f3 = carve(nullptr, conv_x3_pack_floats());
                float* b3 = carve(nullptr, conv_x3_pack_floats());
                if (ws_commit_) { x3_of_[bc_pk_[i]] = f3; x3_of_[bc_pkb_[i]] = b3; }
            }
        }
        bc_Wk4_ = carve(nullptr, 9 * 64 * 4); bc_Wb4_ = carve(nullptr, 9 * 64 * 4);
        bc_dW1r_ = carve(nullptr, (size_t)25 * 64 * D); bc_dWc_ = carve(nullptr, 25 * 64 * 5 + 64);
        bc_dT_ = carve(nullptr, BK * 1600); bc_dM_ = carve(nullptr, BK * 1600); bc_G1_ = carve(nullptr, (size_t)N * 64);
        recon_ = carve("recon", BN * 4);
    } else {
    patches_ = carve("patches", BT * 16 * cfg.obs_channels);
    for (int i = 0; i < 7; ++i) de_[i] = carve(fmt("dvae_enc%d", i).c_str(), BT * 64);
    zraw_ = carve("zraw", BT * V);
    z_ = carve("z", BT * V);
    zdec_ = cfg.hard ? carve("z_st", BT * V) : z_;
    tokens_ = reinterpret_cast<int*>(carve("tokens", BT));
    {
        const size_t nseg = (size_t)gemm_stat_segments(V);
        zstat_ = carve(nullptr, BT * nseg * 2); zhstat_ = carve(nullptr, BT * nseg); zhidx_ = reinterpret_cast<int*>(carve(nullptr, BT * nseg));
        zlse_ = carve("z_lse", BT); zdot_ = carve(nullptr, BT);
        cestat_ = carve(nullptr, BT * nseg * 2); celse_ = carve("ce_lse", BT); cepart_ = carve(nullptr, BT / 16 + 16);
    }
    dd0_ = carve("dvae_dec0", BT * 64); dd1_ = carve("dvae_dec1", BT * 64); dd2_ = carve("dvae_dec2", BT * 64); dd3_ = carve("dvae_dec3", BT * 64);
    dd4_ = carve("dvae_dec4", BT * 256); ps1_ = carve(nullptr, BT * 256);
    dd6_ = carve("dvae_dec6", BT * 256); dd7_ = carve("dvae_dec7", BT * 256); dd8_ = carve("dvae_dec8", BT * 256);
    dd9_ = carve("dvae_dec9", BT * 1024); ps2_ = carve(nullptr, BN * 64);
    recon_ = carve("recon", BN * 4); drecon_ = carve(nullptr, BN * 4);
    for (int i = 0; i < 2; ++i) {
        dw_fwd_[i] = carve(nullptr, 9 * 64 * 64); dw_bwd_[i] = carve(nullptr, 9 * 64 * 64);
        if (conv_x3_ > 0) {
            float* f3 = carve(nullptr, conv_x3_pack_floats(3));
            float* b3 = carve(nullptr, conv_x3_pack_floats(3));
            if (ws_commit_) { x3_of_[dw_fwd_[i]] = f3; x3_of_[dw_bwd_[i]] = b3; }
        }
    }
    w11p_ = carve(nullptr, 4 * 64);
    mem_ = carve("mem", BK * d); emb_ = carve("emb", BT * d);
    for (int b = 0; b < NB; ++b) {
        Blk& k = blk_[b];
        k.ln1 = carve(nullptr, BT * d); k.ln1_mean = carve(nullptr, BT); k.ln1_rstd = carve(nullptr, BT);
        k.q = carve(nullptr, BT * 3 * d); k.k = k.q + d; k.v = k.q + 2 * d;
        k.lse = carve(nullptr, B * NH * (size_t)T); k.ao = carve(nullptr, BT * d); k.x1 = carve(nullptr, BT * d);
        k.ln2 = carve(nullptr, BT * d); k.ln2_mean = carve(nullptr, BT); k.ln2_rstd = carve(nullptr, BT);
        k.cq = carve(nullptr, BT * d); k.ck = carve(nullptr, BK * d); k.cv = carve(nullptr, BK * d);
        k.cP = carve(nullptr, B * NH * (size_t)T * K); k.cao = carve(nullptr, BT * d); k.x2 = carve(nullptr, BT * d);
        k.ln3 = carve(nullptr, BT * d); k.ln3_mean = carve(nullptr, BT); k.ln3_rstd = carve(nullptr, BT);
        k.f1 = carve(fmt("blk%d.ffn_hidden", b).c_str(), BT * 4 * d); k.x3 = carve(nullptr, BT * d);
    }
    bg_.resize(NB);
    {
        const size_t NC = xattn_supported(K, d, NH) ? (size_t)NH * xattn_kp(K, NH) : 16;
        xa_zero_base_ = carve_pos();
        for (int b = 0; b < NB; ++b) {
            Blk& k = blk_[b];
            k.xaAb = carve(nullptr, B * NC * d); k.xaAbT = carve(nullptr, B * NC * d); k.xaVo = carve(nullptr, B * NC * d); k.xaVoT = carve(nullptr, B * NC * d);
        }
        xa_zero_floats_ = (size_t)(carve_pos() - xa_zero_base_);
        for (int b = 0; b < NB; ++b) { bg_[b].xaPd = carve(nullptr, BT * NC); bg_[b].xaDs = carve(nullptr, BT * NC); }
        xa_dAb_ = carve(nullptr, B * NC * d); xa_dVo_ = carve(nullptr, B * NC * d);
        xa_pq_ = carve(nullptr, B * (size_t)d * d); xa_po_ = carve(nullptr, B * (size_t)d * d);
    }
    attn_delta_ = carve(nullptr, B * NH * (size_t)T);
    lnf_ = carve("dec_out", BT * d); lnf_mean_ = carve(nullptr, BT); lnf_rstd_ = carve(nullptr, BT);
    pred_ = carve("pred", BT * V);
    gx_ = carve(nullptr, BT * d); gbr_ = carve(nullptr, BT * d); gt1_ = carve(nullptr, BT * d); gt2_ = carve(nullptr, BT * d);
    gt3_ = carve(nullptr, BT * d); gf1_ = carve(nullptr, BT * 4 * d); gqkv_ = carve(nullptr, BT * 3 * d);
    for (int b = 0; b < NB; ++b) {
        BlkG& q = bg_[b];
        if (b == 0) { q.gbr[0] = gbr_; q.gf1 = gf1_; q.gt2 = gt2_; q.gqkv = gqkv_; }
        else { q.gbr[0] = carve(nullptr, BT * d); q.gf1 = carve(nullptr, BT * 4 * d); q.gt2 = carve(nullptr, BT * d); q.gqkv = carve(nullptr, BT * 3 * d); }
        q.gbr[1] = carve(nullptr, BT * d); q.gbr[2] = carve(nullptr, BT * d);
    }
    scratch3_ = carve(nullptr, scratch_floats_);
    gmem_ = carve(nullptr, BK * d); gck_ = carve(nullptr, BK * d); gcv_ = carve(nullptr, BK * d);
    gdA_ = carve(nullptr, BN * 64); gdB_ = carve(nullptr, BN * 64);
    }
    {
        const int ldc0 = (25 * cfg.obs_channels + 3) & ~3;
        col0_ = carve(nullptr, BN * ldc0); dw0p_ = carve(nullptr, (size_t)64 * ldc0);
    }
    end_layout();
}

int SlateModel::bind(float* p, float* g, float* m, float* v, void* ws, size_t ws_bytes) {
    RC(check_buffers(p, g, ws, ws_bytes));
    OCRL_REQUIRE(d % 64 == 0 && d <= 256 && D % 64 == 0 && C == 64 && V % 256 == 0 && S % 4 == 0 && d % NH == 0 && DH % 4 == 0 && DH <= 64,
                 "unsupported configuration (d_model/slot_size multiples of 64 <= 256, cnn hidden 64, vocab %% 256, obs_size %% 4)");
    OCRL_REQUIRE(cfg.obs_channels == 3, "obs_channels must be 3");
    OCRL_REQUIRE(T % 4 == 0, "obs_size/4 squared must be a multiple of 4");
    adopt_buffers(p, g, m, v, ws);
    clear_encode_graphs();
    packs_valid_ = false;
    layout_workspace(true);
    if (!side_) {
        const char* e = getenv("OCRL_OVERLAP");
        overlap_mode_ = e ? atoi(e) : 5;
        if (overlap_mode_) {
            OCRL_HIP(hipStreamCreateWithFlags(&side_, hipStreamNonBlocking));
            OCRL_HIP(hipEventCreateWithFlags(&ev_fork_, hipEventDisableTiming));
            OCRL_HIP(hipEventCreateWithFlags(&ev_join_, hipEventDisableTiming));
            OCRL_HIP(hipEventCreateWithFlags(&ev_tokens_, hipEventDisableTiming));
            const char* w = getenv("OCRL_DW_SIDE");
            dw_mode_ = (overlap_mode_ >= 3 && !cfg.use_bcdec) ? (w ? atoi(w) : 2) : 0;
            if (dw_mode_) {
                for (hipEvent_t& ev : ev_dw_) OCRL_HIP(hipEventCreateWithFlags(&ev, hipEventDisableTiming));
                OCRL_HIP(hipEventCreateWithFlags(&ev_join2_, hipEventDisableTiming));
                if (dw_mode_ == 2) OCRL_HIP(hipStreamCreateWithFlags(&side2_, hipStreamNonBlocking));
            }
        }
    }
    {
        const char* e = getenv("OCRL_SA_INPUT");
        sa_input_ = e ? atoi(e) : 1;
    }
    {
        const char* e = getenv("OCRL_XATTN");
        xattn_ = !cfg.use_bcdec && xattn_supported(K, d, NH) && (e ? atoi(e) != 0 : true);
        if (!cfg.use_bcdec && xa_zero_floats_) OCRL_HIP(hipMemset(xa_zero_base_, 0, xa_zero_floats_ * sizeof(float)));
    }
    RC(posgrid_launch(gridT_, S, 0));
    RC(fill_launch(recon_, (long long)Bmax * N * 4, 0.f, 0));
    const SaWts wo = sa_wts_layout(C, D, H);
    const SlotAttnW& sa = w_.sa;
    std::vector<PackEntry> ent;
    auto e = [&](ParamRef r, int rows, int cols, int off, int tr) {
        PackEntry x; x.src = P(r); x.rows = rows; x.cols = cols; x.dst_off = off; x.transpose = tr;
        ent.push_back(x);
    };
    e(sa.norm_inputs.w, 1, C, wo.ln_in_g, 0); e(sa.norm_inputs.b, 1, C, wo.ln_in_b, 0);
    e(sa.norm_slots.w, 1, D, wo.ln_s_g, 0); e(sa.norm_slots.b, 1, D, wo.ln_s_b, 0);
    e(sa.norm_mlp.w, 1, D, wo.ln_m_g, 0); e(sa.norm_mlp.b, 1, D, wo.ln_m_b, 0);
    e(sa.q, D, D, wo.Wq, 2); e(sa.q, D, D, wo.WqT, 3);
    e(sa.k, D, C, wo.Wk, 2); e(sa.k, D, C, wo.WkT, 3);
    e(sa.v, D, C, wo.Wv, 2); e(sa.v, D, C, wo.WvT, 3);
    e(sa.gru_wih, 3 * D, D, wo.Wih, 2); e(sa.gru_wih, 3 * D, D, wo.WihT, 3);
    e(sa.gru_whh, 3 * D, D, wo.Whh, 2); e(sa.gru_whh, 3 * D, D, wo.WhhT, 3);
    e(sa.gru_bih, 1, 3 * D, wo.bih, 0); e(sa.gru_bhh, 1, 3 * D, wo.bhh, 0);
    e(sa.m0.w, H, D, wo.W0, 2); e(sa.m0.w, H, D, wo.W0T, 3); e(sa.m0.b, 1, H, wo.b0, 0);
    e(sa.m2.w, D, H, wo.W2, 2); e(sa.m2.w, D, H, wo.W2T, 3); e(sa.m2.b, 1, D, wo.b2, 0);
    sa_pack_n_ = (int)ent.size();
    sa_pack_max_ = 3 * D * D;
    OCRL_REQUIRE(sa_pack_n_ <= 64, "pack table overflow");
    OCRL_HIP(hipMemcpy(sa_pack_dev_, ent.data(), ent.size() * sizeof(PackEntry), hipMemcpyHostToDevice));
    OCRL_HIP(hipDeviceSynchronize());
    have_fwd_ = false;
    return 0;
}

int SlateModel::soft_z(hipStream_t st) {
    if (!fused_heads() || cfg.use_bcdec) return 0;
    OCRL_REQUIRE(have_scores_, "soft_z: no forward since the last backward (the scores have been overwritten by their gradient)");
    return exp_rows_launch(zraw_, zlse_, z_, (long long)last_.B * T, V, st);
}
int SlateModel::dropout_mask(unsigned site, long long n, float* out, hipStream_t st) const {
    return dropout_mask_launch(out, n, pdrop_, last_.seed, site, st);
}

int SlateModel::conv_layer_fwd(const float* x, const float* pack, const float* bias, float* y, int Bn, int Hh, int Ww, int KS, int CIN,
                               int relu, const float* posmap, const float* mask, const Lane& L) {
    ConvArgs a;
    a.X = x; a.Wp = pack; a.Y = y; a.B = Bn; a.H = Hh; a.W = Ww; a.bias = bias; a.relu = relu; a.posmap = posmap; a.mask = mask;
    if (conv_x3_ > 0 && (KS == 5 || KS == 3) && CIN == 64 && !conv_lowlat_) {
        auto it = x3_of_.find(pack);
        if (it != x3_of_.end()) return conv_x3_launch(a, it->second, L, KS);
    }
    return conv_fwd_launch(a, KS, CIN, 64, L, conv_lowlat_);
}
int SlateModel::conv_layer_wgrad(const float* x, const float* dy, float* dW, float* db, int Bn, int Hh, int Ww, int KS, int CIN,
                                 int cin_real, const Lane& L) {
    WgradArgs a;
    a.X = x; a.dY = dy; a.part = L.scratch; a.B = Bn; a.H = Hh; a.W = Ww;
    OCRL_REQUIRE(conv_wgrad_ws_floats(Bn, Hh, Ww, KS, CIN) <= L.scratch_floats, "conv wgrad: scratch too small");
    RC(conv_wgrad_launch(a, KS, CIN, 64, cin_real, dW, 0, L, conv_x3_ > 0 ? 1 : 0));
    if (db) RC(colsum_launch(dy, 64, db, (long long)Bn * Hh * Ww, 64, 0, 1.f, L.scratch, L.scratch_floats, L));
    return 0;
}

int SlateModel::pack_weights(const Lane& L, bool encoder_only) {
    RC(conv_pack_launch(P(w_.enc[0].w), cw_fwd_[0], nullptr, 5, 8, 64, cfg.obs_channels, L));
    RC(conv_pack_launch(P(w_.enc[1].w), cw_fwd_[1], cw_bwd_[1], 5, 64, 64, 64, L));
    RC(conv_pack_launch(P(w_.enc[2].w), cw_fwd_[2], cw_bwd_[2], 5, 64, 64, 64, L));
    RC(conv_pack_launch(P(w_.enc[3].w), cw_fwd_[3], cw_bwd_[3], 5, 64, 64, 64, L));
    if (conv_x3_ > 0) {
        for (int i = 1; i < 4; ++i) {
            auto f = x3_of_.find(cw_fwd_[i]), b = x3_of_.find(cw_bwd_[i]);
            if (f != x3_of_.end()) RC(conv_pack_x3_launch(P(w_.enc[i].w), const_cast<float*>(f->second), b != x3_of_.end() ? const_cast<float*>(b->second) : nullptr, L));
        }
    }
    if (!cfg.use_bcdec && !encoder_only) {
        RC(conv_pack_launch(P(w_.dvae_dec[1].w), dw_fwd_[0], dw_bwd_[0], 3, 64, 64, 64, L));
        RC(conv_pack_launch(P(w_.dvae_dec[6].w), dw_fwd_[1], dw_bwd_[1], 3, 64, 64, 64, L));
        if (conv_x3_ > 0) {
            for (int i = 0; i < 2; ++i) {
                auto f = x3_of_.find(dw_fwd_[i]), b = x3_of_.find(dw_bwd_[i]);
                if (f != x3_of_.end()) RC(conv_pack_x3_launch(P(w_.dvae_dec[i ? 6 : 1].w), const_cast<float*>(f->second), b != x3_of_.end() ? const_cast<float*>(b->second) : nullptr, L, 3));
            }
// ... 263 lines not shown
        OCRL_HIP(hipGraphInstantiate(&eg.exec, g, nullptr, nullptr, 0));
        OCRL_HIP(hipGraphDestroy(g));
    }
    OCRL_HIP(hipGraphLaunch(eg.exec, L));
    return 0;
}

void SlateModel::clear_encode_graphs() {
    for (auto& kv : enc_graphs_) if (kv.second.exec) (void)hipGraphExecDestroy(kv.second.exec);
    enc_graphs_.clear();
}

int SlateModel::encode_backward(const float* dslots, hipStream_t st) {
    OCRL_REQUIRE(have_enc_, "encode_backward: call encode first (its activations are what is differentiated)");
    OCRL_REQUIRE(!frozen_, "encode_backward: the weights are frozen (ocrl_slate_freeze_weights): encode() kept no activations");
    OCRL_REQUIRE(g_ && dslots, "encode_backward: no gradient buffer bound / null dslots");
    const Lane L = main_lane(st);
    RC(fill_launch(g_, flat_size_, 0.f, L));
    RC(copy_launch(dslots, gslots_, (long long)last_.B * K * D, L));
    RC(bwd_encoder(L));
    have_enc_ = false;
    enc_only_grads_ = true;
    return 0;
}

int SlateModel::generate(hipStream_t st) {
    OCRL_REQUIRE(!cfg.use_bcdec, "generate: the autoregressive decoder is not part of the use_bcdec configuration");
    OCRL_REQUIRE(last_.B > 0 && last_.obs, "generate: run forward or encode first");
    have_enc_ = false;
    const int B = last_.B;
    const long long BK = (long long)B * K;
    pdrop_ = 0.f;
    have_fwd_ = false;
    const Lane L = main_lane(st);
    OCRL_HIP(hipMemsetAsync(tokens_, 0, sizeof(int) * (size_t)B * T, L));
    RC(lin_fwd(slots_, D, P(w_.slotproj), nullptr, mem_, d, BK, d, D, 0, nullptr, 0, 0.f, 0, L));
    for (int b = 0; b < NB; ++b) {
        const DecBlockW& bw = w_.blk[b];
        RC(lin_fwd(mem_, d, P(bw.ck), nullptr, blk_[b].ck, d, BK, d, d, 0, nullptr, 0, 0.f, 0, L));
        RC(lin_fwd(mem_, d, P(bw.cv), nullptr, blk_[b].cv, d, BK, d, d, 0, nullptr, 0, 0.f, 0, L));
    }
    float* x0 = emb_;
    for (int t = 0; t < T; ++t) {
        RC(embed_step_launch(tokens_, P(w_.dict), P(w_.bos), P(w_.pe), x0, B, T, d, t, L));
        const float* xin = x0;
        for (int b = 0; b < NB; ++b) {
            Blk& k = blk_[b];
            const DecBlockW& bw = w_.blk[b];
            RC(layernorm_fwd_launch(xin, P(bw.ln1.w), P(bw.ln1.b), k.ln1, k.ln1_mean, k.ln1_rstd, B, d, L));
            const float* res = (b == 0) ? k.ln1 : xin;
            RC(lin_fwd(k.ln1, d, P(bw.qkv), nullptr, k.q + (size_t)t * 3 * d, T * 3 * d, B, 3 * d, d, 0, nullptr, 0, 0.f, 0, L));
            RC(decode_attn_launch(k.q, k.ao, B, T, t, d, NH, 3 * d, L));
            RC(lin_fwd(k.ao, d, P(bw.o), nullptr, k.x1, d, B, d, d, 0, res, d, 0.f, 0, L));
            RC(layernorm_fwd_launch(k.x1, P(bw.ln2.w), P(bw.ln2.b), k.ln2, k.ln2_mean, k.ln2_rstd, B, d, L));
            RC(lin_fwd(k.ln2, d, P(bw.cq), nullptr, k.cq, d, B, d, d, 0, nullptr, 0, 0.f, 0, L));
            RC(cross_attn_fwd_launch(k.cq, k.ck, k.cv, k.cao, k.cP, B, 1, K, d, NH, 0.f, 0, 0, L));
            RC(lin_fwd(k.cao, d, P(bw.co), nullptr, k.x2, d, B, d, d, 0, k.x1, d, 0.f, 0, L));
            RC(layernorm_fwd_launch(k.x2, P(bw.ln3.w), P(bw.ln3.b), k.ln3, k.ln3_mean, k.ln3_rstd, B, d, L));
            RC(lin_fwd(k.ln3, d, P(bw.ffn0.w), P(bw.ffn0.b), k.f1, 4 * d, B, 4 * d, d, 1, nullptr, 0, 0.f, 0, L));
            RC(lin_fwd(k.f1, 4 * d, P(bw.ffn2.w), P(bw.ffn2.b), k.x3, d, B, d, 4 * d, 0, k.x2, d, 0.f, 0, L));
            xin = k.x3;
        }
        RC(layernorm_fwd_launch(xin, P(w_.lnf.w), P(w_.lnf.b), lnf_, lnf_mean_, lnf_rstd_, B, d, L));
        RC(lin_fwd(lnf_, d, P(w_.out), nullptr, pred_, V, B, V, d, 0, nullptr, 0, 0.f, 0, L));
        RC(argmax_pos_launch(pred_, tokens_, B, T, V, t, L, 1));
    }
    RC(onehot_launch(tokens_, z_, (long long)B * T, V, L));
    RC(dvae_decode(B, nullptr, L, z_));
    return 0;
}

int SlateModel::bwd_decoder(const Lane& L) {
    const int B = last_.B;
    const long long BT = (long long)B * T, BK = (long long)B * K;
    const float p = pdrop_;
    const float scale = 1.0f / sqrtf((float)DH);
    const Lane W = dw_lane(L);
    const bool dws = dw_mode_ != 0;
    Xf ce; ce.a_mode = 3; ce.lse = celse_; ce.tok = tokens_; ce.scale = 1.0f / last_.B;
    RC(after(W, L, ring_event()));
    RC(lin_bwd_w(pred_, V, lnf_, d, G(w_.out), nullptr, BT, V, d, 1.f, W, ce));
    RC(lin_bwd_x(pred_, V, P(w_.out), gt1_, d, BT, V, d, nullptr, 0, nullptr, 0, L, Drop(), ce));
    const float* xlast = blk_[NB - 1].x3;
    RC(layernorm_bwd_launch(gt1_, xlast, lnf_mean_, lnf_rstd_, P(w_.lnf.w), gx_, G(w_.lnf.w), BT, d, 0, 0,
                            L.scratch, L.scratch_floats, L));
    RC(fill_launch(gmem_, BK * d, 0.f, L));
    for (int b = NB - 1; b >= 0; --b) {
        Blk& k = blk_[b];
        const BlkG& q = bg_[dws ? b : 0];
        const DecBlockW& bw = w_.blk[b];
        const unsigned site = SITE_BLK_BASE + 8 * b;
        const float* xin = (b == 0) ? emb_ : blk_[b - 1].x3;
        const float* gd = gx_;
        auto drop_gx = [&](unsigned s_, float* into) -> int {
            gd = gx_;
            if (p > 0.f || dws) { RC(dropout_apply_launch(gx_, into, BT * d, p, last_.seed, s_, L)); gd = into; }
            return 0;
        };
        RC(drop_gx(site + 4, q.gbr[0]));
        RC(lin_bwd_x(gd, d, P(bw.ffn2.w), q.gf1, 4 * d, BT, d, 4 * d, k.f1, 4 * d, nullptr, 0, L));
        RC(after(W, L, ring_event()));
        RC(lin_bwd_w(gd, d, k.f1, 4 * d, G(bw.ffn2.w), G(bw.ffn2.b), BT, d, 4 * d, 1.f, W));
        RC(lin_bwd_w(q.gf1, 4 * d, k.ln3, d, G(bw.ffn0.w), G(bw.ffn0.b), BT, 4 * d, d, 1.f, W));
        RC(lin_bwd_x(q.gf1, 4 * d, P(bw.ffn0.w), gt1_, d, BT, 4 * d, d, nullptr, 0, nullptr, 0, L));
        RC(layernorm_bwd_launch(gt1_, k.x2, k.ln3_mean, k.ln3_rstd, P(bw.ln3.w), gx_, G(bw.ln3.w), BT, d, 1, 0,
                                L.scratch, L.scratch_floats, L));
        RC(drop_gx(site + 3, q.gbr[1]));
        const float* gd_co = gd;
        if (xattn_) {
            const int NC = NH * xattn_kp(K, NH);
            XaHost hx = xattn_args(b);
            hx.y = gt1_; hx.gd = gd_co; hx.Pd = q.xaPd; hx.dS = q.xaDs;
            RC(xattn_launch(hx, 1, L));
            RC(after(W, L, ring_event()));
            {
                const int KP = xattn_kp(K, NH), dh = DH;
                const float* Wq = P(bw.cq);
                const float* Wo = P(bw.co);
                GemmArgs ga;
                ga.M = NC; ga.N = d; ga.K = T; ga.lda = NC; ga.ldb = d; ga.ldc = d; ga.akc = 0; ga.bkc = 0; ga.batch = B;
                ga.sA = (long long)T * NC; ga.sB = (long long)T * d; ga.sC = (long long)NC * d;
                ga.A = q.xaPd; ga.B = gd_co; ga.C = xa_dVo_;
                RC(gemm_launch(ga, W));
                ga.A = q.xaDs; ga.B = k.ln2; ga.C = xa_dAb_;
                RC(gemm_launch(ga, W));
                GemmArgs gb;
                gb.M = K; gb.N = dh; gb.K = d; gb.akc = 1; gb.bkc = 1; gb.lda = d; gb.ldb = d; gb.ldc = d; gb.batch = B * NH; gb.batch_inner = NH; gb.alpha = scale;
                gb.A = xa_dAb_; gb.sA = (long long)NC * d; gb.sAi = (long long)KP * d;
                gb.B = Wq; gb.sB = 0; gb.sBi = (long long)dh * d;
                gb.C = gck_; gb.sC = (long long)K * d; gb.sCi = dh;
                RC(gemm_launch(gb, W));
                GemmArgs gc;
                gc.M = K; gc.N = dh; gc.K = d; gc.akc = 1; gc.bkc = 0; gc.lda = d; gc.ldb = d; gc.ldc = d; gc.batch = B * NH; gc.batch_inner = NH;
                gc.A = xa_dVo_; gc.sA = (long long)NC * d; gc.sAi = (long long)KP * d;
                gc.B = Wo; gc.sB = 0; gc.sBi = dh;
                gc.C = gcv_; gc.sC = (long long)K * d; gc.sCi = dh;
                RC(gemm_launch(gc, W));
                GemmArgs gq;
                gq.M = dh; gq.N = d; gq.K = K; gq.akc = 0; gq.bkc = 0; gq.lda = d; gq.ldb = d; gq.ldc = d; gq.batch = B * NH; gq.batch_inner = NH; gq.alpha = scale;
                gq.A = k.ck; gq.sA = (long long)K * d; gq.sAi = dh;
                gq.B = xa_dAb_; gq.sB = (long long)NC * d; gq.sBi = (long long)KP * d;
                gq.C = xa_pq_; gq.sC = (long long)d * d; gq.sCi = (long long)dh * d;
                RC(gemm_launch(gq, W));
                GemmArgs go;
                go.M = d; go.N = dh; go.K = K; go.akc = 0; go.bkc = 0; go.lda = d; go.ldb = d; go.ldc = d; go.batch = B * NH; go.batch_inner = NH;
                go.A = xa_dVo_; go.sA = (long long)NC * d; go.sAi = (long long)KP * d;
                go.B = k.cv; go.sB = (long long)K * d; go.sBi = dh;
                go.C = xa_po_; go.sC = (long long)d * d; go.sCi = dh;
                RC(gemm_launch(go, W));
                RC(colsum_launch(xa_pq_, (long long)d * d, G(bw.cq), B, d * d, 0, 1.f, W.scratch, W.scratch_floats, W));
                RC(colsum_launch(xa_po_, (long long)d * d, G(bw.co), B, d * d, 0, 1.f, W.scratch, W.scratch_floats, W));
            }
        } else {
        RC(lin_bwd_x(gd, d, P(bw.co), gt1_, d, BT, d, d, nullptr, 0, nullptr, 0, L));
        RC(cross_attn_bwd_launch(gt1_, k.cq, k.ck, k.cv, k.cP, q.gt2, gck_, gcv_, B, T, K, d, NH, p, last_.seed, site + 2, L.scratch, L.scratch_floats, L));
        RC(after(W, L, ring_event()));
        RC(lin_bwd_w(gd_co, d, k.cao, d, G(bw.co), nullptr, BT, d, d, 1.f, W));
        RC(lin_bwd_w(q.gt2, d, k.ln2, d, G(bw.cq), nullptr, BT, d, d, 1.f, W));
        RC(lin_bwd_x(q.gt2, d, P(bw.cq), gt1_, d, BT, d, d, nullptr, 0, nullptr, 0, L));
        }
        {
            const Lane& X = xattn_ ? W : L;
            RC(lin_bwd_w(gck_, d, mem_, d, G(bw.ck), nullptr, BK, d, d, 1.f, X));
            RC(lin_bwd_w(gcv_, d, mem_, d, G(bw.cv), nullptr, BK, d, d, 1.f, X));
            RC(lin_bwd_x(gck_, d, P(bw.ck), gmem_, d, BK, d, d, nullptr, 0, gmem_, d, X));
            RC(lin_bwd_x(gcv_, d, P(bw.cv), gmem_, d, BK, d, d, nullptr, 0, gmem_, d, X));
        }
        RC(layernorm_bwd_launch(gt1_, k.x1, k.ln2_mean, k.ln2_rstd, P(bw.ln2.w), gx_,
                                G(bw.ln2.w), BT, d, 1, 0, L.scratch, L.scratch_floats, L));
        RC(drop_gx(site + 1, q.gbr[2]));
        const float* gd_o = gd;
        RC(lin_bwd_x(gd, d, P(bw.o), gt1_, d, BT, d, d, nullptr, 0, nullptr, 0, L));
        {
            AttnArgs a = self_attn_args(b);
            a.dO = gt1_; a.dq = q.gqkv; a.dk = q.gqkv + d; a.dv = q.gqkv + 2 * d; a.delta = attn_delta_;
            RC(attn_launch(a, 1, L));
        }
        RC(after(W, L, ring_event()));
        RC(lin_bwd_w(gd_o, d, k.ao, d, G(bw.o), nullptr, BT, d, d, 1.f, W));
        RC(lin_bwd_w(q.gqkv, 3 * d, k.ln1, d, G(bw.qkv), nullptr, BT, 3 * d, d, 1.f, W));
        RC(lin_bwd_x(q.gqkv, 3 * d, P(bw.qkv), gt1_, d, BT, 3 * d, d, nullptr, 0, nullptr, 0, L));
        if (b == 0) {
            RC(axpy_launch(gx_, gt1_, BT * d, 1.f, L));
            RC(layernorm_bwd_launch(gt1_, xin, k.ln1_mean, k.ln1_rstd, P(bw.ln1.w), gx_,
                                    G(bw.ln1.w), BT, d, 0, 0, L.scratch, L.scratch_floats, L));
        } else {
            RC(layernorm_bwd_launch(gt1_, xin, k.ln1_mean, k.ln1_rstd, P(bw.ln1.w), gx_,
                                    G(bw.ln1.w), BT, d, 1, 0, L.scratch, L.scratch_floats, L));
        }
    }
    RC(embed_bwd_launch(gx_, tokens_, G(w_.dict), B, T, V, d, p, last_.seed, L.scratch, L.scratch_floats, L));
    RC(fill_launch(G(w_.pe), (long long)(T + 1) * d, 0.f, L));
    RC(colsum_launch(gx_, (long long)T * d, G(w_.pe), B, T * d, 0, 1.f, L.scratch, L.scratch_floats, L));
    RC(copy_launch(G(w_.pe), G(w_.bos), d, L));
    if (xattn_) RC(after(L, W, ring_event()));
    RC(lin_bwd_w(gmem_, d, slots_, D, G(w_.slotproj), nullptr, BK, d, D, 1.f, L));
    RC(lin_bwd_x(gmem_, d, P(w_.slotproj), gslots_, D, BK, d, D, nullptr, 0, nullptr, 0, L));
    return 0;
}

int SlateModel::bwd_encoder(const Lane& L, bool fork_dvae) {
    const int B = last_.B;
    const long long BN = (long long)B * N, R = (long long)B * I * K;
    const SaSave so = sa_save_layout(C, D, H, SH);
    const SaGrad go = sa_grad_layout(C, D, H, SH);
    const SlotAttnW& sa = w_.sa;
    SlotAttnArgs a;
    a.B = B; a.N = N; a.C = C; a.K = K; a.D = D; a.H = H; a.I = I; a.NH = SH; a.eps = 1e-8f; a.scale = 1.0f / sqrtf((float)(D / SH));
    a.x = x_; a.wts = sa_wts_; a.save = sa_save_; a.dslots = gslots_; a.dx = gA_; a.dslots0 = gslots0_; a.grows = sa_grows_; a.g_small = sa_small_;
    a.xchg = sa_xchg_; a.parts = sa_parts_;
    if (fork_dvae) {
        RC(after(dvae_lane(), L, ev_fork_));
        RC(bwd_dvae(dvae_lane()));
    }
    RC(slot_attn_launch(a, 1, L));
    const bool side_w = side_ && overlap_mode_ >= 3 && !cfg.use_bcdec && !fork_dvae;
    const Lane W = side_w ? dvae_lane() : L;
    if (side_w) RC(after(W, L, ev_fork_));
    const bool sa_in_bwd = sa_input_ == 1 && C == 64;
    RC(lin_bwd_w(sa_grows_ + go.out, go.ld, sa_save_ + so.hid, so.ld, G(sa.m2.w), G(sa.m2.b), R, D, H, 1.f, W));
    RC(lin_bwd_w(sa_grows_ + go.hid, go.ld, sa_save_ + so.m, so.ld, G(sa.m0.w), G(sa.m0.b), R, H, D, 1.f, W));
    RC(lin_bwd_w(sa_grows_ + go.gi, go.ld, sa_save_ + so.u, so.ld, G(sa.gru_wih), G(sa.gru_bih), R, 3 * D, D, 1.f, W));
    RC(lin_bwd_w(sa_grows_ + go.gh, go.ld, sa_save_ + so.sprev, so.ld, G(sa.gru_whh), G(sa.gru_bhh), R, 3 * D, D, 1.f, W));
    RC(lin_bwd_w(sa_grows_ + go.q, go.ld, sa_save_ + so.sn, so.ld, G(sa.q), nullptr, R, D, D, 1.f, W));
    for (int h = 0, dh = D / SH; h < SH; ++h) {
        RC(lin_bwd_w(sa_grows_ + go.u + h * dh, go.ld, sa_save_ + so.up + h * C, so.ld, G(sa.v) + (size_t)h * dh * C, nullptr, R, dh, C, 1.f, W));
        RC(lin_bwd_w(sa_save_ + so.q + h * dh, so.ld, sa_grows_ + go.qp + h * C, go.ld, G(sa.k) + (size_t)h * dh * C, nullptr, R, dh, C, a.scale, W));
    }
    const int SM = 4 * D + 2 * C;
    RC(colsum_launch(sa_small_ + 0, SM, G(sa.norm_slots.w), B, 2 * D, 0, 1.f, W.scratch, W.scratch_floats, W));
    RC(colsum_launch(sa_small_ + 2 * D, SM, G(sa.norm_mlp.w), B, 2 * D, 0, 1.f, W.scratch, W.scratch_floats, W));
    RC(colsum_launch(sa_small_ + 4 * D, SM, G(sa.norm_inputs.w), B, 2 * C, 0, 1.f, W.scratch, W.scratch_floats, W));
    RC(slot_init_bwd_launch(gslots0_, P(w_.sa.log_sigma), last_.noise_slots, G(w_.sa.mu), G(w_.sa.log_sigma),
                            B * K, D, last_.seed, W));
    if (!sa_in_bwd) RC(lin_bwd_w(gA_, C, h1_, C, G(w_.sa.mlp2.w), G(w_.sa.mlp2.b), BN, C, C, 1.f, W));
    if (side_w) RC(im2col5_launch(obs8_, col0_, BN, S, S, cfg.obs_channels, (25 * cfg.obs_channels + 3) & ~3, W));
    if (sa_in_bwd) {
        const size_t slabs = L.scratch_floats / SA_INPUT_SLAB;
        OCRL_REQUIRE(slabs >= 1, "bwd_encoder: scratch too small for the input-chain slabs");
        RC(sa_input_bwd_launch(gA_, h1_, e4_, ln0_mean_, ln0_rstd_, P(w_.sa.ln.w), P(w_.sa.ln.b),
                               P(w_.sa.mlp0.w), P(w_.sa.mlp2.w), gB_, G(w_.sa.mlp0.w), G(w_.sa.mlp0.b),
                               G(w_.sa.mlp2.w), G(w_.sa.mlp2.b), G(w_.sa.ln.w), G(w_.sa.ln.b),
                               BN, slabs < 512 ? (int)slabs : 0, L.scratch, L.scratch_floats, L));
    } else {
        RC(lin_bwd_x(gA_, C, P(w_.sa.mlp2.w), gB_, C, BN, C, C, h1_, C, nullptr, 0, L));
        RC(lin_bwd_w(gB_, C, ln0_, C, G(w_.sa.mlp0.w), G(w_.sa.mlp0.b), BN, C, C, 1.f, L));
        float* gL = side_w ? gC_ : gA_;
        RC(lin_bwd_x(gB_, C, P(w_.sa.mlp0.w), gL, C, BN, C, C, nullptr, 0, nullptr, 0, L));
        RC(layernorm_bwd_launch(gL, e4_, ln0_mean_, ln0_rstd_, P(w_.sa.ln.w), gB_, G(w_.sa.ln.w), BN, C, 0, 0,
                                L.scratch, L.scratch_floats, L));
    }
    RC(colsum_launch(gB_, (long long)N * C, gmap_, B, N * C, 0, 1.f, L.scratch, L.scratch_floats, L));
    RC(lin_bwd_w(gmap_, C, gridT_, 4, G(w_.enc_pos.w), G(w_.enc_pos.b), N, C, 4, 1.f, L));
    if (fork_dvae || side_w) RC(after(L, dvae_lane(), ev_join_));
    if (dw_mode_ == 2 && side2_) RC(after(L, dw_lane(L), ev_join2_));
    RC(colsum_launch(gmap_, C, G(w_.enc[3].b), N, C, 0, 1.f, L.scratch, L.scratch_floats, L));
    RC(conv_layer_wgrad(e3_, gB_, G(w_.enc[3].w), nullptr, B, S, S, 5, 64, 64, L));
    RC(conv_layer_fwd(gB_, cw_bwd_[3], nullptr, gA_, B, S, S, 5, 64, 0, nullptr, e3_, L));
    RC(conv_layer_wgrad(e2_, gA_, G(w_.enc[2].w), G(w_.enc[2].b), B, S, S, 5, 64, 64, L));
    RC(conv_layer_fwd(gA_, cw_bwd_[2], nullptr, gB_, B, S, S, 5, 64, 0, nullptr, e2_, L));
    RC(conv_layer_wgrad(e1_, gB_, G(w_.enc[1].w), G(w_.enc[1].b), B, S, S, 5, 64, 64, L));
    RC(conv_layer_fwd(gB_, cw_bwd_[1], nullptr, gA_, B, S, S, 5, 64, 0, nullptr, e1_, L));
    {
        const int ch = cfg.obs_channels, ldc0 = (25 * ch + 3) & ~3;
        if (!side_w) RC(im2col5_launch(obs8_, col0_, BN, S, S, ch, ldc0, L));
        RC(lin_bwd_w(gA_, 64, col0_, ldc0, dw0p_, G(w_.enc[0].b), BN, 64, ldc0, 1.f, L));
        RC(unpack5_launch(dw0p_, G(w_.enc[0].w), ch, ldc0, L));
    }
    return 0;
}

int SlateModel::bwd_dvae(const Lane& L) {
// ... 180 lines not shown
```

ocrl_amd/csrc/slate_model.h:

```cpp
#pragma once
#include <map>
#include <string>
#include <vector>

#include "kernels.h"
#include "model_base.h"

struct SlateConfig {
    int obs_size = 64, obs_channels = 3, vocab = 4096, d_model = 192, cnn_hidden = 64;
    int num_slots = 5, num_iters = 3, slot_size = 192, mlp_hidden = 192;
    int num_blocks = 4, num_heads = 4;
    float dropout = 0.1f;
    int max_batch = 1;
    int use_bcdec = 0;
    int hard = 0;
    int slot_heads = 1;
};

struct StepInputs {
    const float* obs = nullptr;
    int B = 0;
    float tau = 1.f;
    int train = 1;
    unsigned long long seed = 0;
// ... 43 lines not shown
    int conv_layer_fwd(const float* x, const float* pack, const float* bias, float* y, int Bn, int Hh, int Ww, int KS, int CIN, int relu,
                       const float* posmap, const float* mask, const Lane& L);
    int conv_layer_wgrad(const float* x, const float* dy, float* dW, float* db, int Bn, int Hh, int Ww, int KS, int CIN, int cin_real,
                         const Lane& L);
    int pack_weights(const Lane& L, bool encoder_only = false);
    int fwd_encoder(const StepInputs& in, const Lane& L, int fork_dvae = 0);
    int fwd_dvae(const StepInputs& in, const Lane& L);
    int fwd_decoder(const Lane& L, bool with_ce = true);
    int dvae_decode(int B, float* drecon, const Lane& L, const float* zin = nullptr);
    int bwd_decoder(const Lane& L);
    int bwd_encoder(const Lane& L, bool fork_dvae = false);
    int bwd_dvae(const Lane& L);
    int pack_bcdec(const Lane& L);
    int fwd_bcdec(const Lane& L);
    int bwd_bcdec(const Lane& L);
    AttnArgs self_attn_args(int b) const;
    XaHost xattn_args(int b) const;

    Lane main_lane(hipStream_t st) const { return Lane{st, scratch_, scratch_floats_}; }
    Lane dvae_lane() const { return Lane{side_, scratch2_, scratch_floats_}; }
    Lane dw_lane(const Lane& main) const { return dw_mode_ == 2 ? Lane{side2_, scratch3_, scratch_floats_} : dw_mode_ ? dvae_lane() : main; }
    int after(const Lane& waiter, const Lane& producer, hipEvent_t ev);
    hipEvent_t ring_event() { return ev_dw_[ev_dw_next_++ & 7]; }

    struct DecBlockW { ParamPair ln1, ln2, ln3, ffn0, ffn2; ParamRef qkv, o, cq, ck, cv, co; };
    struct SlotAttnW {
        ParamRef mu, log_sigma, q, k, v, gru_wih, gru_whh, gru_bih, gru_bhh;
        ParamPair ln, mlp0, mlp2, norm_inputs, norm_slots, norm_mlp, m0, m2;
    };
    struct Weights {
        ParamPair dvae_enc[8], dvae_dec[12];
        ParamPair enc[4], enc_pos;
        SlotAttnW sa;
        ParamPair bc[4], bc_pos;
        ParamRef slotproj, dict, bos, pe, out;
        ParamPair lnf;
        std::vector<DecBlockW> blk;
        long long enc_grads_end = 0;
    } w_;
    void resolve_params();

    long long group_begin_[4] = {0, 0, 0, 0};

    int S, E, T, N, V, d, C, K, I, D, H, NB, NH, DH, Bmax;
    int SH = 1;
    StepInputs last_;
    float pdrop_ = 0.f;
    bool have_fwd_ = false;
    int conv_lowlat_ = 0;
    bool frozen_ = false, packs_valid_ = false;
    bool have_enc_ = false;
    bool enc_only_grads_ = false;
    bool have_scores_ = false;

    float *scratch_ = nullptr;
    size_t scratch_floats_ = 0;
    float* scratch2_ = nullptr;
    int overlap_mode_ = 0;
    hipStream_t side_ = nullptr;
    hipEvent_t ev_fork_ = nullptr, ev_join_ = nullptr, ev_tokens_ = nullptr;
    float *zstat_ = nullptr, *zhstat_ = nullptr, *zlse_ = nullptr, *zdot_ = nullptr, *cestat_ = nullptr, *celse_ = nullptr, *cepart_ = nullptr;
    int* zhidx_ = nullptr;
    float *obs8_, *patches_, *de_[7], *zraw_, *z_, *zdec_;
    int* tokens_;
    float *dd0_, *dd1_, *dd2_, *dd3_, *dd4_, *ps1_, *dd6_, *dd7_, *dd8_, *dd9_, *ps2_, *recon_, *drecon_;
    float *e1_, *e2_, *e3_, *e4_, *posmap_, *gridT_, *ln0_, *ln0_mean_, *ln0_rstd_, *h1_, *x_;
    float *slots0_, *slot_noise_, *slots_, *attn_, *sa_save_, *sa_wts_, *sa_grows_, *sa_small_, *sa_xchg_;
    float* attn_heads_ = nullptr;
    float* sa_parts_;
    PackEntry* sa_pack_dev_ = nullptr;
    int sa_pack_n_ = 0, sa_pack_max_ = 0;
    float *cw_fwd_[4], *cw_bwd_[4];
    int conv_x3_ = -1;
    std::map<const float*, const float*> x3_of_;
    float *dw_fwd_[2], *dw_bwd_[2];
    float *w11p_;
    float *mem_, *emb_;
    struct Blk {
        float *ln1, *ln1_mean, *ln1_rstd, *q, *k, *v, *lse, *ao, *x1;
        float *ln2, *ln2_mean, *ln2_rstd, *cq, *ck, *cv, *cP, *cao, *x2;
        float *ln3, *ln3_mean, *ln3_rstd, *f1, *x3;
        float *xaAb, *xaAbT, *xaVo, *xaVoT;
    };
    int sa_input_ = 1;
    bool xattn_ = false;
    float *xa_dAb_ = nullptr, *xa_dVo_ = nullptr, *xa_pq_ = nullptr, *xa_po_ = nullptr;
    size_t xa_zero_floats_ = 0;
    float* xa_zero_base_ = nullptr;
    std::vector<Blk> blk_;
    struct BlkG { float *gbr[3], *gf1, *gt2, *gqkv, *xaPd, *xaDs; };
    std::vector<BlkG> bg_;
    struct EncGraph { hipGraphExec_t exec = nullptr; int warm = 0; };
    std::map<int, EncGraph> enc_graphs_;
    int enc_graph_mode_ = -1;
    hipStream_t cap_ = nullptr;
    float* obs_stage_ = nullptr;
    unsigned long long* seed_dev_ = nullptr;
    int dw_mode_ = 0;
    hipStream_t side2_ = nullptr;
    float* scratch3_ = nullptr;
    hipEvent_t ev_dw_[8] = {nullptr, nullptr, nullptr, nullptr, nullptr, nullptr, nullptr, nullptr};
    hipEvent_t ev_join2_ = nullptr;
    int ev_dw_next_ = 0;
    float *attn_delta_;
    float *lnf_, *lnf_mean_, *lnf_rstd_, *pred_;
    float *gqkv_;
    float *gx_, *gbr_, *gt1_, *gt2_, *gt3_, *gf1_, *gmem_, *gck_, *gcv_, *gslots_, *gslots0_;
    float *gA_, *gB_, *gC_;
    float *gdA_, *gdB_;
    float *gmap_;
    float *col0_, *dw0p_;
    float *bc_Wc_, *bc_W1r_, *bc_P1_, *bc_M_, *bc_T_, *bc_c1_, *bc_c2_, *bc_c3_, *bc_out4_, *bc_dout4_, *bc_gA_, *bc_gB_;
    float *bc_pk_[2], *bc_pkb_[2], *bc_Wk4_, *bc_Wb4_, *bc_dW1r_, *bc_dWc_, *bc_dT_, *bc_dM_, *bc_G1_;
};
```

Before: 1733.

## Fuse decoder layernorm backward with dropout and defer gamma/beta reductions into one batched pass

In the transformer decoder backward, each layernorm backward now writes per-block partial tables and, in the same kernel, applies the following gradient dropout and adds the residual gradient. This replaces separate dropout_apply and axpy launches. All per-site gamma/beta column reductions are deferred to a single batched reduce launch after the block loop instead of one colsum pair per layernorm. The goal is fewer launches and fewer passes over the BT x d gradient, at the cost of extra table workspace. The path is skipped when the bcdec decoder is used.

```diff
diff --git a/include/ocrl_hip.h b/include/ocrl_hip.h
--- a/include/ocrl_hip.h
+++ b/include/ocrl_hip.h
@@ -107,6 +107,14 @@
 int ocrl_layernorm_fwd(const float* x, const float* gamma, const float* beta, float* y, float* mean, float* rstd, long long R, int F, void* stream);
 int ocrl_layernorm_bwd(const float* dy, const float* x, const float* mean, const float* rstd, const float* gamma, float* dx, float* dgb,
                        long long R, int F, float* ws, size_t ws_floats, void* stream);
+size_t ocrl_layernorm_bwd_table_floats(long long R, int F);
+int ocrl_layernorm_bwd_site(float* dy, const float* dy2, const float* x, const float* mean, const float* rstd, const float* gamma, float* dx,
+                            float* ydrop, long long R, int F, int accumulate_dx, float p, unsigned long long seed, unsigned site, float* table,
+                            size_t table_floats, void* stream);
+size_t ocrl_layernorm_bwd_reduce_ws_floats(int n, int F);
+int ocrl_layernorm_bwd_reduce(const float* const* tables, float* const* dgb, const long long* rows, int n, int F, int accumulate_dgb, float* ws,
+                              size_t ws_floats, void* stream);
+int ocrl_dropout_apply(const float* x, float* y, long long n, float p, unsigned long long seed, unsigned site, void* stream);
 
 int ocrl_sa_input_plan(long long R, int out[3]);
 int ocrl_sa_input_fwd(const float* e4, const float* gamma, const float* beta, const float* W0, const float* b0, const float* W2, const float* b2,
diff --git a/ocrl_amd/_lib.py b/ocrl_amd/_lib.py
--- a/ocrl_amd/_lib.py
+++ b/ocrl_amd/_lib.py
@@ -157,6 +157,13 @@
     L.ocrl_conv2d_bwd_weight_ex.argtypes = [POINTER(ConvWgradDesc), p, c_size_t, p]
     L.ocrl_layernorm_fwd.argtypes = [p, p, p, p, p, p, c_longlong, c_int, p]
     L.ocrl_layernorm_bwd.argtypes = [p, p, p, p, p, p, p, c_longlong, c_int, p, c_size_t, p]
+    L.ocrl_layernorm_bwd_table_floats.argtypes = [c_longlong, c_int]
+    L.ocrl_layernorm_bwd_table_floats.restype = c_size_t
+    L.ocrl_layernorm_bwd_site.argtypes = [p] * 8 + [c_longlong, c_int, c_int, c_float, c_ulonglong, c_uint, p, c_size_t, p]
+    L.ocrl_layernorm_bwd_reduce_ws_floats.argtypes = [c_int, c_int]
+    L.ocrl_layernorm_bwd_reduce_ws_floats.restype = c_size_t
+    L.ocrl_layernorm_bwd_reduce.argtypes = [POINTER(p), POINTER(p), POINTER(c_longlong), c_int, c_int, c_int, p, c_size_t, p]
+    L.ocrl_dropout_apply.argtypes = [p, p, c_longlong, c_float, c_ulonglong, c_uint, p]
     L.ocrl_sa_input_plan.argtypes = [c_longlong, POINTER(c_int * 3)]
     L.ocrl_sa_input_fwd.argtypes = [p] * 11 + [c_longlong, c_int, p]
     L.ocrl_sa_input_bwd.argtypes = [p] * 16 + [c_longlong, c_int, p, c_size_t, p]
diff --git a/ocrl_amd/csrc/capi.cpp b/ocrl_amd/csrc/capi.cpp
--- a/ocrl_amd/csrc/capi.cpp
+++ b/ocrl_amd/csrc/capi.cpp
@@ -299,6 +299,32 @@
                        int F, float* ws, size_t ws_floats, void* stream) {
     return layernorm_bwd_launch(dy, x, mean, rstd, g, dx, dgb, R, F, 0, 0, ws, ws_floats, ST(stream));
 }
+size_t ocrl_layernorm_bwd_table_floats(long long R, int F) { return R > 0 && F > 0 ? ln_site_table_floats(R, F) : 0; }
+int ocrl_layernorm_bwd_site(float* dy, const float* dy2, const float* x, const float* mean, const float* rstd, const float* g, float* dx, float* ydrop,
+                            long long R, int F, int accumulate_dx, float p, unsigned long long seed, unsigned site, float* table, size_t table_floats,
+                            void* stream) {
+    if (!dy || !x || !mean || !rstd || !g || !dx || !table || R < 1) { ocrl_set_error("ocrl_layernorm_bwd_site: dy, x, mean, rstd, gamma, dx, table and R >= 1 are required"); return 1; }
+    LnSiteArgs s;
+    s.dy2 = dy2; s.ydrop = ydrop; s.p = p; s.seed = seed; s.site = site;
+    return layernorm_bwd_site_launch(dy, x, mean, rstd, g, dx, R, F, accumulate_dx ? 1 : 0, s, table, table_floats, ST(stream));
+}
+size_t ocrl_layernorm_bwd_reduce_ws_floats(int n, int F) { return n > 0 && F > 0 ? (size_t)n * LN_REDUCE_CHUNKS * 2 * F : 0; }
+int ocrl_layernorm_bwd_reduce(const float* const* tables, float* const* dgb, const long long* rows, int n, int F, int accumulate_dgb, float* ws,
+                              size_t ws_floats, void* stream) {
+    if (!tables || !dgb || !rows || n < 1 || n > LN_SITES_MAX) { ocrl_set_error("ocrl_layernorm_bwd_reduce: tables, dgb, rows and 1..%d sites are required", LN_SITES_MAX); return 1; }
+    LnReduce r;
+    r.n = n; r.F = F;
+    for (int i = 0; i < n; ++i) {
+        if (rows[i] < 1) { ocrl_set_error("ocrl_layernorm_bwd_reduce: rows[%d] = %lld", i, rows[i]); return 1; }
+        r.table[i] = tables[i]; r.dgb[i] = dgb[i]; r.nblk[i] = ln_site_nblk(rows[i]);
+    }
+    return layernorm_bwd_reduce_launch(r, accumulate_dgb ? 1 : 0, ws, ws_floats, ST(stream));
+}
+int ocrl_dropout_apply(const float* x, float* y, long long n, float p, unsigned long long seed, unsigned site, void* stream) {
+    if (!x || !y || n < 0 || !(p >= 0.f && p < 1.f)) { ocrl_set_error("ocrl_dropout_apply: x, y, n >= 0 and p in [0, 1) are required"); return 1; }
+    if (n == 0) return 0;
+    return dropout_apply_launch(x, y, n, p, seed, site, ST(stream));
+}
 
 int ocrl_sa_input_plan(long long R, int out[3]) {
     if (!out || R <= 0) { ocrl_set_error("ocrl_sa_input_plan: needs R > 0 and an output array"); return 1; }
diff --git a/ocrl_amd/csrc/elementwise.hip b/ocrl_amd/csrc/elementwise.hip
--- a/ocrl_amd/csrc/elementwise.hip
+++ b/ocrl_amd/csrc/elementwise.hip
@@ -180,9 +180,9 @@
     }
 }
 template <int NV, int NP>
-__global__ __launch_bounds__(256) void layernorm16_bwd_kernel(const float* __restrict__ dy, const float* __restrict__ x, const float* __restrict__ mean,
-                                                              const float* __restrict__ rstd, const float* __restrict__ g, float* __restrict__ dx,
-                                                              float* __restrict__ part, long long R, int accumulate) {
+__global__ __launch_bounds__(256) void layernorm16_bwd_kernel(const float* dy, const float* __restrict__ x, const float* __restrict__ mean,
+                                                              const float* __restrict__ rstd, const float* __restrict__ g, float* dx,
+                                                              float* __restrict__ part, long long R, int accumulate, LnSiteArgs s) {
     constexpr int F = 64 * NV;
     __shared__ float4 red[2][16][16 * NV];
     const int lane = threadIdx.x & 63, wv = threadIdx.x >> 6, c4 = lane & 15, rsub = lane >> 4;
@@ -201,6 +201,10 @@
             for (int k = 0; k < NV; ++k) {
                 xv[i][k] = ok ? *reinterpret_cast<const float4*>(x + row * F + (k * 16 + c4) * 4) : make_float4(0.f, 0.f, 0.f, 0.f);
                 yv[i][k] = ok ? *reinterpret_cast<const float4*>(dy + row * F + (k * 16 + c4) * 4) : make_float4(0.f, 0.f, 0.f, 0.f);
+                if (s.dy2 && ok) {
+                    const float4 b = *reinterpret_cast<const float4*>(s.dy2 + row * F + (k * 16 + c4) * 4);
+                    yv[i][k].x += b.x; yv[i][k].y += b.y; yv[i][k].z += b.z; yv[i][k].w += b.w;
+                }
             }
             mu[i] = ok ? mean[row] : 0.f;
             rs[i] = ok ? rstd[row] : 0.f;
@@ -216,6 +220,19 @@
                     float* dp = dx + row * F + (k * 16 + c4) * 4;
                     if (accumulate) { const float4 a = *reinterpret_cast<const float4*>(dp); o.x += a.x; o.y += a.y; o.z += a.z; o.w += a.w; }
                     *reinterpret_cast<float4*>(dp) = o;
+                    if (s.ydrop) {
+                        const long long i4 = row * (F / 4) + k * 16 + c4;
+                        if (s.p > 0.f) {
+                            const uint2 bits = rng_bits4(s.seed, s.site, (uint64_t)i4);
+                            const uint32_t thr = drop_thresh(s.p);
+                            const float sc = 1.0f / (1.0f - s.p);
+                            o.x = rng_keep(bits, 0, thr) ? o.x * sc : 0.f;
+                            o.y = rng_keep(bits, 1, thr) ? o.y * sc : 0.f;
+                            o.z = rng_keep(bits, 2, thr) ? o.z * sc : 0.f;
+                            o.w = rng_keep(bits, 3, thr) ? o.w * sc : 0.f;
+                        }
+                        *reinterpret_cast<float4*>(s.ydrop + i4 * 4) = o;
+                    }
                 }
             }
         }
@@ -232,24 +249,28 @@
     }
 }
 
-__global__ void colsum_kernel(const float* __restrict__ X, long long ld, float* __restrict__ part, long long R, int F, long long rows_per_chunk) {
+__device__ __forceinline__ void colsum_body(const float* __restrict__ X, long long ld, float* __restrict__ part, long long R, int F, long long rows_per_chunk,
+                                            int colblk, int chunk) {
     __shared__ float red[4][64];
-    const int col = blockIdx.x * 64 + (threadIdx.x & 63), rl = threadIdx.x >> 6;
-    const long long r0 = (long long)blockIdx.y * rows_per_chunk;
+    const int col = colblk * 64 + (threadIdx.x & 63), rl = threadIdx.x >> 6;
+    const long long r0 = (long long)chunk * rows_per_chunk;
     const long long r1 = min(R, r0 + rows_per_chunk);
     float s = 0.f;
     if (col < F)
         for (long long r = r0 + rl; r < r1; r += 4) s += X[r * ld + col];
     red[rl][threadIdx.x & 63] = s;
     __syncthreads();
-    if (rl == 0 && col < F) part[(size_t)blockIdx.y * F + col] = red[0][threadIdx.x] + red[1][threadIdx.x] + red[2][threadIdx.x] + red[3][threadIdx.x];
-}
-__global__ __launch_bounds__(256) void colsum4_kernel(const float* __restrict__ X, long long ld, float* __restrict__ part, long long R, int F,
-                                                      long long rows_per_chunk) {
+    if (rl == 0 && col < F) part[(size_t)chunk * F + col] = red[0][threadIdx.x] + red[1][threadIdx.x] + red[2][threadIdx.x] + red[3][threadIdx.x];
+}
+__global__ void colsum_kernel(const float* __restrict__ X, long long ld, float* __restrict__ part, long long R, int F, long long rows_per_chunk) {
+    colsum_body(X, ld, part, R, F, rows_per_chunk, blockIdx.x, blockIdx.y);
+}
+__device__ __forceinline__ void colsum4_body(const float* __restrict__ X, long long ld, float* __restrict__ part, long long R, int F,
+                                             long long rows_per_chunk, int chunk) {
     __shared__ float4 red[256];
     const int F4 = F >> 2, RL = 256 / F4;
     const int c4 = threadIdx.x % F4, rl = threadIdx.x / F4;
-    const long long r0 = (long long)blockIdx.x * rows_per_chunk;
+    const long long r0 = (long long)chunk * rows_per_chunk;
     const long long r1 = min(R, r0 + rows_per_chunk);
     float4 s0 = make_float4(0.f, 0.f, 0.f, 0.f), s1 = s0, s2 = s0, s3 = s0;
     if (rl < RL) {
@@ -273,13 +294,18 @@
     if (threadIdx.x < F4) {
         float4 t = red[threadIdx.x];
         for (int k = 1; k < RL; ++k) { const float4 v = red[k * F4 + threadIdx.x]; t.x += v.x; t.y += v.y; t.z += v.z; t.w += v.w; }
-        *reinterpret_cast<float4*>(part + (size_t)blockIdx.x * F + threadIdx.x * 4) = t;
-    }
-}
-__global__ __launch_bounds__(256) void colsum_final_kernel(const float* __restrict__ part, float* __restrict__ out, int nchunk, int F, int accumulate, float scale) {
+        *reinterpret_cast<float4*>(part + (size_t)chunk * F + threadIdx.x * 4) = t;
+    }
+}
+__global__ __launch_bounds__(256) void colsum4_kernel(const float* __restrict__ X, long long ld, float* __restrict__ part, long long R, int F,
+                                                      long long rows_per_chunk) {
+    colsum4_body(X, ld, part, R, F, rows_per_chunk, blockIdx.x);
+}
+__device__ __forceinline__ void colsum_final_body(const float* __restrict__ part, float* __restrict__ out, int nchunk, int F, int accumulate, float scale,
+                                                  int colblk) {
     __shared__ float red[16][16];
     const int cl = threadIdx.x & 15, rl = threadIdx.x >> 4;
-    const int c = blockIdx.x * 16 + cl;
+    const int c = colblk * 16 + cl;
     float s0 = 0.f, s1 = 0.f;
     if (c < F) {
         int k = rl;
@@ -295,6 +321,24 @@
         t *= scale;
         out[c] = accumulate ? out[c] + t : t;
     }
+}
+__global__ __launch_bounds__(256) void colsum_final_kernel(const float* __restrict__ part, float* __restrict__ out, int nchunk, int F, int accumulate, float scale) {
+    colsum_final_body(part, out, nchunk, F, accumulate, scale, blockIdx.x);
+}
+__global__ __launch_bounds__(256) void colsum_sites_kernel(LnReduce r, float* __restrict__ ws, size_t stride) {
+    const int y = blockIdx.y, F2 = 2 * r.F;
+    const ColsumPlan pl = r.plan[y];
+    float* part = ws + (size_t)y * stride;
+    if (pl.mode == 4) {
+        if ((long long)blockIdx.x < pl.nchunk) colsum4_body(r.table[y], F2, part, r.nblk[y], F2, pl.rpc, blockIdx.x);
+    } else {
+        const int cb = (F2 + 63) / 64;
+        if ((long long)blockIdx.x < pl.nchunk * cb) colsum_body(r.table[y], F2, part, r.nblk[y], F2, pl.rpc, blockIdx.x % cb, blockIdx.x / cb);
+    }
+}
+__global__ __launch_bounds__(256) void colsum_final_sites_kernel(LnReduce r, const float* __restrict__ ws, size_t stride, int accumulate) {
+    const int y = blockIdx.y;
+    colsum_final_body(ws + (size_t)y * stride, r.dgb[y], (int)r.plan[y].nchunk, 2 * r.F, accumulate, 1.f, blockIdx.x);
 }
 
 __global__ void reduce_partials_kernel(const float* __restrict__ part, int n, float* __restrict__ out, float scale, int accumulate) {
@@ -1202,19 +1246,17 @@
     OCRL_CHECK_LAUNCH("layernorm_fwd");
     return 0;
 }
-int colsum_launch(const float* X, long long ld, float* out, long long R, int F, int accumulate, float scale, float* ws, size_t ws_floats, hipStream_t st) {
+ColsumPlan colsum_plan(const float* X, long long ld, long long R, int F, size_t ws_floats) {
+    ColsumPlan pl;
     if (F % 4 == 0 && ld % 4 == 0 && F <= 1024 && F >= 4 && (((uintptr_t)X) & 15) == 0 && R >= 1024) {
         long long nchunk = 2048;
         if (nchunk > R / 8) nchunk = R / 8;
         if ((size_t)nchunk * F > ws_floats) nchunk = (long long)(ws_floats / F);
         if (nchunk >= 16) {
-            const long long rpc = (R + nchunk - 1) / nchunk;
-            nchunk = (R + rpc - 1) / rpc;
-            hipLaunchKernelGGL(colsum4_kernel, dim3((unsigned)nchunk), dim3(256), 0, st, X, ld, ws, R, F, rpc);
-            OCRL_CHECK_LAUNCH("colsum4");
-            hipLaunchKernelGGL(colsum_final_kernel, dim3(cdiv(F, 16)), dim3(256), 0, st, ws, out, (int)nchunk, F, accumulate, scale);
-            OCRL_CHECK_LAUNCH("colsum_final");
-            return 0;
+            pl.mode = 4;
+            pl.rpc = (R + nchunk - 1) / nchunk;
+            pl.nchunk = (R + pl.rpc - 1) / pl.rpc;
+            return pl;
         }
     }
     const int cb = cdiv(F, 64);
@@ -1222,38 +1264,87 @@
     if (nchunk < 1) nchunk = 1;
     if (nchunk > (R + 63) / 64) nchunk = (R + 63) / 64;
     if (nchunk < 1) nchunk = 1;
-    OCRL_REQUIRE((size_t)nchunk * F <= ws_floats, "colsum: workspace too small (%lld x %d)", nchunk, F);
-    const long long rpc = (R + nchunk - 1) / nchunk;
-    hipLaunchKernelGGL(colsum_kernel, dim3(cb, (int)nchunk), dim3(256), 0, st, X, ld, ws, R, F, rpc);
-    OCRL_CHECK_LAUNCH("colsum");
-    hipLaunchKernelGGL(colsum_final_kernel, dim3(cdiv(F, 16)), dim3(256), 0, st, ws, out, (int)nchunk, F, accumulate, scale);
+    pl.mode = (size_t)nchunk * F <= ws_floats ? 1 : 0;
+    pl.nchunk = nchunk;
+    pl.rpc = (R + nchunk - 1) / nchunk;
+    return pl;
+}
+int colsum_launch(const float* X, long long ld, float* out, long long R, int F, int accumulate, float scale, float* ws, size_t ws_floats, hipStream_t st) {
+    const ColsumPlan pl = colsum_plan(X, ld, R, F, ws_floats);
+    if (pl.mode == 4) {
+        hipLaunchKernelGGL(colsum4_kernel, dim3((unsigned)pl.nchunk), dim3(256), 0, st, X, ld, ws, R, F, pl.rpc);
+        OCRL_CHECK_LAUNCH("colsum4");
+    } else {
+        OCRL_REQUIRE(pl.mode == 1, "colsum: workspace too small (%lld x %d)", pl.nchunk, F);
+        hipLaunchKernelGGL(colsum_kernel, dim3(cdiv(F, 64), (int)pl.nchunk), dim3(256), 0, st, X, ld, ws, R, F, pl.rpc);
+        OCRL_CHECK_LAUNCH("colsum");
+    }
+    hipLaunchKernelGGL(colsum_final_kernel, dim3(cdiv(F, 16)), dim3(256), 0, st, ws, out, (int)pl.nchunk, F, accumulate, scale);
     OCRL_CHECK_LAUNCH("colsum_final");
+    return 0;
+}
+static int layernorm_bwd_rows(const float* dy, const float* x, const float* mean, const float* rstd, const float* g, float* dx, float* part, int nblk,
+                              long long R, int F, int accumulate_dx, const LnSiteArgs& s, hipStream_t st) {
+    dim3 grid(nblk), blk(256);
+    const bool al16 = aligned16(x, dy, dx, g, part, s.dy2, s.ydrop) && (F == 64 || F == 192);
+    switch (F / 64) {
+        case 1:
+            if (al16) hipLaunchKernelGGL((layernorm16_bwd_kernel<1, 4>), grid, blk, 0, st, dy, x, mean, rstd, g, dx, part, R, accumulate_dx, s);
+            else hipLaunchKernelGGL(layernorm_bwd_kernel<1>, grid, blk, 0, st, dy, x, mean, rstd, g, dx, part, R, accumulate_dx);
+            break;
+        case 2: hipLaunchKernelGGL(layernorm_bwd_kernel<2>, grid, blk, 0, st, dy, x, mean, rstd, g, dx, part, R, accumulate_dx); break;
+        case 3:
+            if (al16) hipLaunchKernelGGL((layernorm16_bwd_kernel<3, 2>), grid, blk, 0, st, dy, x, mean, rstd, g, dx, part, R, accumulate_dx, s);
+            else hipLaunchKernelGGL(layernorm_bwd_kernel<3>, grid, blk, 0, st, dy, x, mean, rstd, g, dx, part, R, accumulate_dx);
+            break;
+        default: hipLaunchKernelGGL(layernorm_bwd_kernel<4>, grid, blk, 0, st, dy, x, mean, rstd, g, dx, part, R, accumulate_dx); break;
+    }
+    OCRL_CHECK_LAUNCH("layernorm_bwd");
     return 0;
 }
 int layernorm_bwd_launch(const float* dy, const float* x, const float* mean, const float* rstd, const float* g, float* dx,
                          float* dgb, long long R, int F, int accumulate_dx, int accumulate_dgb, float* ws, size_t ws_floats, hipStream_t st) {
     OCRL_REQUIRE(F % 64 == 0 && F >= 64 && F <= 256, "layernorm bwd: F must be 64..256, multiple of 64 (got %d)", F);
-    int nblk = (int)((R + 3) / 4);
-    if (nblk > 2048) nblk = 2048;
+    int nblk = ln_site_nblk(R);
     while (nblk > 64 && (size_t)nblk * 2 * F * 2 + (size_t)8 * 2 * F > ws_floats) nblk /= 2;
     const size_t need = (size_t)nblk * 2 * F;
     OCRL_REQUIRE(need + (size_t)8 * 2 * F <= ws_floats, "layernorm bwd: workspace too small");
-    dim3 grid(nblk), blk(256);
-    const bool al16 = aligned16(x, dy, dx, g, ws);
-    switch (F / 64) {
-        case 1:
-            if (al16) hipLaunchKernelGGL((layernorm16_bwd_kernel<1, 4>), grid, blk, 0, st, dy, x, mean, rstd, g, dx, ws, R, accumulate_dx);
-            else hipLaunchKernelGGL(layernorm_bwd_kernel<1>, grid, blk, 0, st, dy, x, mean, rstd, g, dx, ws, R, accumulate_dx);
-            break;
-        case 2: hipLaunchKernelGGL(layernorm_bwd_kernel<2>, grid, blk, 0, st, dy, x, mean, rstd, g, dx, ws, R, accumulate_dx); break;
-        case 3:
-            if (al16) hipLaunchKernelGGL((layernorm16_bwd_kernel<3, 2>), grid, blk, 0, st, dy, x, mean, rstd, g, dx, ws, R, accumulate_dx);
-            else hipLaunchKernelGGL(layernorm_bwd_kernel<3>, grid, blk, 0, st, dy, x, mean, rstd, g, dx, ws, R, accumulate_dx);
-            break;
-        default: hipLaunchKernelGGL(layernorm_bwd_kernel<4>, grid, blk, 0, st, dy, x, mean, rstd, g, dx, ws, R, accumulate_dx); break;
-    }
-    OCRL_CHECK_LAUNCH("layernorm_bwd");
+    RC(layernorm_bwd_rows(dy, x, mean, rstd, g, dx, ws, nblk, R, F, accumulate_dx, LnSiteArgs(), st));
     return colsum_launch(ws, 2 * F, dgb, nblk, 2 * F, accumulate_dgb, 1.f, ws + need, ws_floats - need, st);
+}
+int layernorm_bwd_site_launch(float* dy, const float* x, const float* mean, const float* rstd, const float* g, float* dx, long long R, int F,
+                              int accumulate_dx, const LnSiteArgs& s, float* table, size_t table_floats, hipStream_t st) {
+    OCRL_REQUIRE(F % 64 == 0 && F >= 64 && F <= 256, "layernorm bwd: F must be 64..256, multiple of 64 (got %d)", F);
+    OCRL_REQUIRE(R >= 1 && table && ln_site_table_floats(R, F) <= table_floats, "layernorm bwd site: table of %zu floats, %zu needed", table_floats,
+                 ln_site_table_floats(R, F));
+    OCRL_REQUIRE(!s.ydrop || (s.p >= 0.f && s.p < 1.f), "layernorm bwd site: dropout p %g outside [0, 1)", (double)s.p);
+    const int nblk = ln_site_nblk(R);
+    if (aligned16(x, dy, dx, g, table, s.dy2, s.ydrop) && (F == 64 || F == 192))
+        return layernorm_bwd_rows(dy, x, mean, rstd, g, dx, table, nblk, R, F, accumulate_dx, s, st);
+    if (s.dy2) RC(axpy_launch(s.dy2, dy, R * F, 1.f, st));
+    RC(layernorm_bwd_rows(dy, x, mean, rstd, g, dx, table, nblk, R, F, accumulate_dx, LnSiteArgs(), st));
+    if (s.ydrop) RC(dropout_apply_launch(dx, s.ydrop, R * F, s.p, s.seed, s.site, st));
+    return 0;
+}
+int layernorm_bwd_reduce_launch(LnReduce r, int accumulate_dgb, float* ws, size_t ws_floats, hipStream_t st) {
+    if (r.n == 0) return 0;
+    OCRL_REQUIRE(r.n > 0 && r.n <= LN_SITES_MAX, "layernorm bwd reduce: 1..%d sites (got %d)", LN_SITES_MAX, r.n);
+    OCRL_REQUIRE(r.F % 64 == 0 && r.F >= 64 && r.F <= 256, "layernorm bwd reduce: F must be 64..256, multiple of 64 (got %d)", r.F);
+    const size_t stride = (size_t)LN_REDUCE_CHUNKS * 2 * r.F;
+    OCRL_REQUIRE(ws && stride * r.n <= ws_floats, "layernorm bwd reduce: workspace of %zu floats, %zu needed", ws_floats, stride * r.n);
+    long long gx = 1;
+    for (int i = 0; i < r.n; ++i) {
+        OCRL_REQUIRE(r.table[i] && r.dgb[i] && r.nblk[i] >= 1 && r.nblk[i] <= 2048, "layernorm bwd reduce: site %d needs a table, dgb and 1..2048 partial rows", i);
+        r.plan[i] = colsum_plan(r.table[i], 2 * r.F, r.nblk[i], 2 * r.F, stride);
+        OCRL_REQUIRE(r.plan[i].mode != 0 && r.plan[i].nchunk <= LN_REDUCE_CHUNKS, "layernorm bwd reduce: site %d: %lld chunks", i, r.plan[i].nchunk);
+        const long long blocks = r.plan[i].mode == 4 ? r.plan[i].nchunk : r.plan[i].nchunk * cdiv(2 * r.F, 64);
+        if (blocks > gx) gx = blocks;
+    }
+    hipLaunchKernelGGL(colsum_sites_kernel, dim3((unsigned)gx, r.n), dim3(256), 0, st, r, ws, stride);
+    OCRL_CHECK_LAUNCH("colsum_sites");
+    hipLaunchKernelGGL(colsum_final_sites_kernel, dim3(cdiv(2 * r.F, 16), r.n), dim3(256), 0, st, r, (const float*)ws, stride, accumulate_dgb);
+    OCRL_CHECK_LAUNCH("colsum_final_sites");
+    return 0;
 }
 int reduce_partials_launch(const float* part, int n, float* out, float scale, int accumulate, hipStream_t st) {
     hipLaunchKernelGGL(reduce_partials_kernel, dim3(1), dim3(256), 0, st, part, n, out, scale, accumulate);
diff --git a/ocrl_amd/csrc/kernels.h b/ocrl_amd/csrc/kernels.h
--- a/ocrl_amd/csrc/kernels.h
+++ b/ocrl_amd/csrc/kernels.h
@@ -227,6 +227,28 @@
 int layernorm_bwd_launch(const float* dy, const float* x, const float* mean, const float* rstd, const float* g, float* dx,
                          float* dgb, long long R, int F, int accumulate_dx, int accumulate_dgb, float* ws, size_t ws_floats, hipStream_t st);
 int colsum_launch(const float* X, long long ld, float* out, long long R, int F, int accumulate, float scale, float* ws, size_t ws_floats, hipStream_t st);
+struct ColsumPlan { int mode = 0; long long nchunk = 0, rpc = 0; };
+ColsumPlan colsum_plan(const float* X, long long ld, long long R, int F, size_t ws_floats);
+struct LnSiteArgs {
+    const float* dy2 = nullptr;
+    float* ydrop = nullptr;
+    float p = 0.f;
+    unsigned long long seed = 0;
+    unsigned site = 0;
+};
+inline int ln_site_nblk(long long R) { return R + 3 >= 4 * 2048 ? 2048 : (int)((R + 3) / 4); }
+inline size_t ln_site_table_floats(long long R, int F) { return (size_t)ln_site_nblk(R) * 2 * F; }
+int layernorm_bwd_site_launch(float* dy, const float* x, const float* mean, const float* rstd, const float* g, float* dx, long long R, int F,
+                              int accumulate_dx, const LnSiteArgs& s, float* table, size_t table_floats, hipStream_t st);
+constexpr int LN_SITES_MAX = 16, LN_REDUCE_CHUNKS = 256;
+struct LnReduce {
+    int n = 0, F = 0;
+    const float* table[LN_SITES_MAX] = {};
+    float* dgb[LN_SITES_MAX] = {};
+    int nblk[LN_SITES_MAX] = {};
+    ColsumPlan plan[LN_SITES_MAX];
+};
+int layernorm_bwd_reduce_launch(LnReduce r, int accumulate_dgb, float* ws, size_t ws_floats, hipStream_t st);
 
 #define SA_INPUT_SLAB (2 * 4096 + 4 * 64)
 void sa_input_plan(long long R, int max_wgs, int out[3]);
diff --git a/ocrl_amd/csrc/slate_model.cpp b/ocrl_amd/csrc/slate_model.cpp
--- a/ocrl_amd/csrc/slate_model.cpp
+++ b/ocrl_amd/csrc/slate_model.cpp
@@ -263,6 +263,8 @@
         q.gbr[1] = carve(nullptr, BT * d); q.gbr[2] = carve(nullptr, BT * d);
     }
     scratch3_ = carve(nullptr, scratch_floats_);
+    ln_tab_ = carve(nullptr, (size_t)(1 + 3 * NB) * ln_site_table_floats((long long)BT, d));
+    ln_red_ws_ = carve(nullptr, (size_t)(1 + 3 * NB) * LN_REDUCE_CHUNKS * 2 * d);
     gmem_ = carve(nullptr, BK * d); gck_ = carve(nullptr, BK * d); gcv_ = carve(nullptr, BK * d);
     gdA_ = carve(nullptr, BN * 64); gdB_ = carve(nullptr, BN * 64);
     }
@@ -303,6 +305,18 @@
     {
         const char* e = getenv("OCRL_SA_INPUT");
         sa_input_ = e ? atoi(e) : 1;
+    }
+    {
+        const char* e = getenv("OCRL_LN_SITE");
+        ln_site_ = (e ? atoi(e) != 0 : true) && !cfg.use_bcdec && 1 + 3 * NB <= LN_SITES_MAX;
+        ln_red_ = LnReduce();
+        if (ln_site_) {
+            const size_t tab = ln_site_table_floats((long long)Bmax * T, d);
+            auto site = [&](const ParamPair& ln) { ln_red_.table[ln_red_.n] = ln_tab_ + ln_red_.n * tab; ln_red_.dgb[ln_red_.n] = G(ln.w); ++ln_red_.n; };
+            ln_red_.F = d;
+            site(w_.lnf);
+            for (int b = 0; b < NB; ++b) { site(w_.blk[b].ln3); site(w_.blk[b].ln2); site(w_.blk[b].ln1); }
+        }
     }
     {
         const char* e = getenv("OCRL_XATTN");
@@ -732,8 +746,18 @@
     RC(lin_bwd_w(pred_, V, lnf_, d, G(w_.out), nullptr, BT, V, d, 1.f, W, ce));
     RC(lin_bwd_x(pred_, V, P(w_.out), gt1_, d, BT, V, d, nullptr, 0, nullptr, 0, L, Drop(), ce));
     const float* xlast = blk_[NB - 1].x3;
-    RC(layernorm_bwd_launch(gt1_, xlast, lnf_mean_, lnf_rstd_, P(w_.lnf.w), gx_, G(w_.lnf.w), BT, d, 0, 0,
-                            L.scratch, L.scratch_floats, L));
+    const size_t ln_tab = ln_site_table_floats((long long)Bmax * T, d);
+    auto ln_bwd = [&](int idx, const float* x, const float* mean, const float* rstd, const ParamPair& ln, int acc, bool add_gx, unsigned dsite, float* into) -> int {
+        if (ln_site_) {
+            LnSiteArgs s;
+            s.dy2 = add_gx ? gx_ : nullptr;
+            if (into && (p > 0.f || dws)) { s.ydrop = into; s.p = p; s.seed = last_.seed; s.site = dsite; }
+            return layernorm_bwd_site_launch(gt1_, x, mean, rstd, P(ln.w), gx_, BT, d, acc, s, ln_tab_ + idx * ln_tab, ln_tab, L);
+        }
+        if (add_gx) RC(axpy_launch(gx_, gt1_, BT * d, 1.f, L));
+        return layernorm_bwd_launch(gt1_, x, mean, rstd, P(ln.w), gx_, G(ln.w), BT, d, acc, 0, L.scratch, L.scratch_floats, L);
+    };
+    RC(ln_bwd(0, xlast, lnf_mean_, lnf_rstd_, w_.lnf, 0, false, SITE_BLK_BASE + 8 * (NB - 1) + 4, bg_[dws ? NB - 1 : 0].gbr[0]));
     RC(fill_launch(gmem_, BK * d, 0.f, L));
     for (int b = NB - 1; b >= 0; --b) {
         Blk& k = blk_[b];
@@ -744,7 +768,10 @@
         const float* gd = gx_;
         auto drop_gx = [&](unsigned s_, float* into) -> int {
             gd = gx_;
-            if (p > 0.f || dws) { RC(dropout_apply_launch(gx_, into, BT * d, p, last_.seed, s_, L)); gd = into; }
+            if (p > 0.f || dws) {
+                if (!ln_site_) RC(dropout_apply_launch(gx_, into, BT * d, p, last_.seed, s_, L));
+                gd = into;
+            }
             return 0;
         };
         RC(drop_gx(site + 4, q.gbr[0]));
@@ -753,8 +780,7 @@
         RC(lin_bwd_w(gd, d, k.f1, 4 * d, G(bw.ffn2.w), G(bw.ffn2.b), BT, d, 4 * d, 1.f, W));
         RC(lin_bwd_w(q.gf1, 4 * d, k.ln3, d, G(bw.ffn0.w), G(bw.ffn0.b), BT, 4 * d, d, 1.f, W));
         RC(lin_bwd_x(q.gf1, 4 * d, P(bw.ffn0.w), gt1_, d, BT, 4 * d, d, nullptr, 0, nullptr, 0, L));
-        RC(layernorm_bwd_launch(gt1_, k.x2, k.ln3_mean, k.ln3_rstd, P(bw.ln3.w), gx_, G(bw.ln3.w), BT, d, 1, 0,
-                                L.scratch, L.scratch_floats, L));
+        RC(ln_bwd(1 + 3 * b, k.x2, k.ln3_mean, k.ln3_rstd, bw.ln3, 1, false, site + 3, q.gbr[1]));
         RC(drop_gx(site + 3, q.gbr[1]));
         const float* gd_co = gd;
         if (xattn_) {
@@ -816,8 +842,7 @@
             RC(lin_bwd_x(gck_, d, P(bw.ck), gmem_, d, BK, d, d, nullptr, 0, gmem_, d, X));
             RC(lin_bwd_x(gcv_, d, P(bw.cv), gmem_, d, BK, d, d, nullptr, 0, gmem_, d, X));
         }
-        RC(layernorm_bwd_launch(gt1_, k.x1, k.ln2_mean, k.ln2_rstd, P(bw.ln2.w), gx_,
-                                G(bw.ln2.w), BT, d, 1, 0, L.scratch, L.scratch_floats, L));
+        RC(ln_bwd(2 + 3 * b, k.x1, k.ln2_mean, k.ln2_rstd, bw.ln2, 1, false, site + 1, q.gbr[2]));
         RC(drop_gx(site + 1, q.gbr[2]));
         const float* gd_o = gd;
         RC(lin_bwd_x(gd, d, P(bw.o), gt1_, d, BT, d, d, nullptr, 0, nullptr, 0, L));
@@ -831,13 +856,15 @@
         RC(lin_bwd_w(q.gqkv, 3 * d, k.ln1, d, G(bw.qkv), nullptr, BT, 3 * d, d, 1.f, W));
         RC(lin_bwd_x(q.gqkv, 3 * d, P(bw.qkv), gt1_, d, BT, 3 * d, d, nullptr, 0, nullptr, 0, L));
         if (b == 0) {
-            RC(axpy_launch(gx_, gt1_, BT * d, 1.f, L));
-            RC(layernorm_bwd_launch(gt1_, xin, k.ln1_mean, k.ln1_rstd, P(bw.ln1.w), gx_,
-                                    G(bw.ln1.w), BT, d, 0, 0, L.scratch, L.scratch_floats, L));
+            RC(ln_bwd(3 + 3 * b, xin, k.ln1_mean, k.ln1_rstd, bw.ln1, 0, true, 0, nullptr));
         } else {
-            RC(layernorm_bwd_launch(gt1_, xin, k.ln1_mean, k.ln1_rstd, P(bw.ln1.w), gx_,
-                                    G(bw.ln1.w), BT, d, 1, 0, L.scratch, L.scratch_floats, L));
-        }
+            RC(ln_bwd(3 + 3 * b, xin, k.ln1_mean, k.ln1_rstd, bw.ln1, 1, false, site - 8 + 4, bg_[dws ? b - 1 : 0].gbr[0]));
+        }
+    }
+    if (ln_site_) {
+        LnReduce r = ln_red_;
+        for (int i = 0; i < r.n; ++i) r.nblk[i] = ln_site_nblk(BT);
+        RC(layernorm_bwd_reduce_launch(r, 0, ln_red_ws_, (size_t)r.n * LN_REDUCE_CHUNKS * 2 * d, L));
     }
     RC(embed_bwd_launch(gx_, tokens_, G(w_.dict), B, T, V, d, p, last_.seed, L.scratch, L.scratch_floats, L));
     RC(fill_launch(G(w_.pe), (long long)(T + 1) * d, 0.f, L));
diff --git a/ocrl_amd/csrc/slate_model.h b/ocrl_amd/csrc/slate_model.h
--- a/ocrl_amd/csrc/slate_model.h
+++ b/ocrl_amd/csrc/slate_model.h
@@ -149,6 +149,9 @@
         float *ln3, *ln3_mean, *ln3_rstd, *f1, *x3;
         float *xaAb, *xaAbT, *xaVo, *xaVoT;
     };
+    int ln_site_ = 1;
+    float *ln_tab_ = nullptr, *ln_red_ws_ = nullptr;
+    LnReduce ln_red_;
     int sa_input_ = 1;
     bool xattn_ = false;
     float *xa_dAb_ = nullptr, *xa_dVo_ = nullptr, *xa_pq_ = nullptr, *xa_po_ = nullptr;
```

After: 1736 (median of 6 runs). Within noise of the previous version (+0.2%).
